# QueensGambit/CrazyAra

Hardware: AMD Instinct MI355X
Metric: nn_evals_per_sec (higher is better)
Workload: dtype f16x3; 1 GPU; crazyhouse RISEv2 19-block (34x8x8 planes -> 5184 policy + value), batch=256, inputs resident in HBM, random-init seeded weights; batch=256, parallelism=replicas x1, precision=float16x3

## Files before the change

crazyara_amd/csrc/nn/kernels.h:

```cpp
#pragma once
#include <hip/hip_runtime.h>
#include <cstdint>

namespace cra {

typedef _Float16 half_t;

constexpr int kSquares = 64;

inline int64_t packed_weight_elems(int cout_pad, int k_total) { return int64_t(cout_pad) * k_total; }

struct ConvArgs {
    const void* x;
    const void* wpk;
    const void* wpk_lo;
    const float* bias;
    const void* resid;
    void* out;
    int batch;
    int cin;
    int cout_pad;
    int cout_real;
    int cout_ld;
    int ks;
    int relu;
    int out_policy_f32;
    int out_flat;
    int flat_pitch;
    int out_rows_f32;
    int rows_valid;
    float* softmax_out;
    const float* planes;
    int planes_c;
    int p8;
    float acc_scale;
    const void *pre_wpk, *pre_wpk_lo;
    const float* pre_bias;
    float pre_acc_scale;
    int dev;
    int few_boards;
    int x_ld;
};

template <typename T> void launch_conv_gemm(const ConvArgs& a, hipStream_t s);

struct BlockArgs {
    const void* x;
    void* y;
    const void* w1pk;
    const float* b1;
    const float* wdw;
    const float* b2;
    const void* w3pk;
    const void* w1pk_lo;
    const void* w3pk_lo;
    const float* b3;
    int batch, C, cop_pad, ks;
    const float* gate;
    float* pool_out;
    const float* dwpk;
};
template <typename T> void launch_block(const BlockArgs& a, hipStream_t s);
void launch_conv_gemm_x3(const ConvArgs& a, hipStream_t s);
void launch_block_x3(const BlockArgs& a, hipStream_t s);
void init_x3_kernel_attributes();
int block_x3_chunk_channels();
struct X3TowerBlock {
    const void *w1pk, *w1pk_lo, *w3pk, *w3pk_lo;
    const float* dwpk;
    const float* b3;
    const float* se_w1t;
    const float* se_w2t;
    const float* se_b;
    int cop_pad;
    int se_kind;
    float w1_inv, w3_scale, w3_inv;
};
struct X3TowerArgs {
    const float* x;
    float* y;
    const X3TowerBlock* blocks;
    int nblocks;
    int batch;
    int p8;
    int ks;
    int symmetric;
};
void launch_tower_x3(const X3TowerArgs& a, hipStream_t s);
struct X3SplitArgs {
    X3TowerBlock blk;
    const float* x_parts;
    float* y_parts;
    int gin;
    int batch, G;
    const float* pool_in;
    float* pool_out;
    int dev;
};
void launch_block_x3_split(const X3SplitArgs& a, hipStream_t s);
void launch_x3_split_finish(const float* parts, int gin, float* y, int batch, hipStream_t s);
template <typename T> void init_block_kernel_attributes();
template <typename T> int block_chunk_channels();

constexpr int kTowerWindow = 16;
struct TowerBlockDesc {
    const float* b3;
    const float* s3;
    const void* se_w1;
    const void* se_w2;
    const float* se_b;
    int cop_pad;
    int ks;
    int se_kind;
    float qx_inv, qt_inv, escale;
};
struct TowerArgs {
    const void* x;
    void* y;
    const TowerBlockDesc* blocks;
    const void* wstream;
    const float* bstream;
    const void* pstream;
    long long wstream_wave_frags, bstream_wave_floats, pstream_wave_bytes;
    int nblocks;
    int batch;
    const float* gate_in;
    float* pool_out;
    unsigned long long* trace;
    int fp8;
    long long wstream_e_frags;
    void* block_dump;
};
void launch_tower(const TowerArgs& a, hipStream_t s);
void init_tower_kernel_attributes();
size_t tower_lds_bytes();
inline int tower_row_of_position(int p) { return (p % 4) + 8 * ((p % 16) / 4) + 4 * (p / 16); }
inline int tower_k_channel(int kpos) {
    const int chunk = kpos / 128, wq = (kpos % 128) / 32, p = kpos % 32;
    return chunk * 128 + wq * 32 + tower_row_of_position(p);
}

struct StemArgs {
    const float* planes;
    void* x;
    const void* stem_w;
    const float* stem_b;
    long long stem_wave_frags;
    int cin, cin_pad;
    int batch;
    const void* descs;
    int layout, n_valid;
};
void launch_stem(const StemArgs& a, hipStream_t s);

struct HeadArgs {
    const void* x;
    float* logits;
    float* probs;
    float* value;
    float* aux;
    const void* s1;
    const float* b1;
    const void* s2;
    long long s1_wave_frags, s2_wave_frags;
    const float* vconv_bias;
    const void* fc1_w;
    const float* fc1_b;
    const float* fc2_w;
    float fc2_b;
    float wdl_b[4];
    int cp;
    int wdlp;
    int batch;
    unsigned long long* trace;
    const uint16_t* g_idx;
    const uint32_t* g_cnt;
    float* g_out;
    int g_stride, g_n_valid;
};
void launch_head(const HeadArgs& a, hipStream_t s);
void init_head_kernel_attributes();
size_t head_lds_bytes();

void launch_forward(const StemArgs& sa, const TowerArgs& ta, const HeadArgs& ha, hipStream_t s);
void init_forward_kernel_attributes();

struct ResTowerArgs {
    const void* x;
    void* y;
    const void* wstream;
    const float* bstream;
    long long wstream_wave_frags;
    long long bstream_wave_floats;
    int nblocks;
    int relu_after_add;
    int batch;
    int boards_per_workgroup;
    int cout_tiles_per_wave;
};
void launch_restower(const ResTowerArgs& a, hipStream_t s);
void init_restower_kernel_attributes();
size_t restower_lds_bytes();

template <typename T> void launch_depthwise(const T* x, T* y, const float* w, const float* bias, int batch, int C, int ks,
                                            hipStream_t s);

template <typename T> void launch_se(T* x, int kind_flags, const float* w1t, const float* w2t, const float* b1, int batch, int C,
                                     hipStream_t s, const T* res = nullptr);

void launch_se_gate(const float* pool, float* gate, int kind, const float* w1t, const float* w2t, const float* b1, int batch, int C,
                    hipStream_t s);

struct ValueHeadArgs {
    const void* x;
    const float* wconv;
    const float* bconv;
    const float* w1t;
    const float* b1;
    const float* w2;
    float b2;
    const float* wwdl;
    const float* bwdl;
    const float* wplys;
    float bplys;
    float* value;
    float* aux;
    int batch, C, cv, fc;
    float* dbg;
    int lds_pad;
    int variant;
};
template <typename T> void prepare_value_head(const ValueHeadArgs& a);
size_t value_head_lds_bytes(const ValueHeadArgs& a);
template <typename T> void launch_value_head(const ValueHeadArgs& a, hipStream_t s);

struct HeadsSmallArgs {
    ConvArgs conv;
    ValueHeadArgs vh;
};
bool heads_small_fits(const ConvArgs& c, const ValueHeadArgs& v);
void launch_heads_small(const HeadsSmallArgs& a, hipStream_t s);
// ... 38 lines not shown
```

crazyara_amd/csrc/nn/precision.cpp:

```cpp
#include <cstdlib>
#include <stdexcept>

#include "rise_net.h"

namespace cra {

namespace {
constexpr bool kX3ValueHeadOneLaunch = true;
}

RiseNet::DevSwitches::DevSwitches() {
    if (const char* e = getenv("CRA_X3_CONV_DEV")) conv_dev = atoi(e);
    device_graph = getenv("CRA_DEVICE_GRAPH") != nullptr;
    lane_graph = getenv("CRA_LANE_GRAPH") != nullptr;
    lane_no_graph = getenv("CRA_LANE_NO_GRAPH") != nullptr;
    predict_copy = getenv("CRA_PREDICT_COPY") != nullptr;
    predict_zero_copy = getenv("CRA_PREDICT_ZERO_COPY") != nullptr;
    if (const char* e = getenv("CRA_LANE_LAUNCHES")) lane_launches = e[0];
    lane_sync = getenv("CRA_LANE_SYNC") != nullptr;
    if (const char* e = getenv("CRA_X3_TOWER")) x3_symmetric = e[0] == 's';
    if (const char* e = getenv("CRA_X3_SPLIT_DEV")) x3_split_dev = atoi(e);
    no_small_path = getenv("CRA_NO_SMALL_PATH") != nullptr;
    if (const char* e = getenv("CRA_SMALL_BATCH_CONV_SPLIT")) small_conv_split = atoi(e);
    tower_trace = getenv("CRA_TOWER_TRACE") != nullptr;
    x3_value_one_launch = kX3ValueHeadOneLaunch;
    if (const char* e = getenv("CRA_X3_VALUE_HEAD")) x3_value_one_launch = e[0] == 'o';
    value_head_debug = getenv("CRA_VALUE_HEAD_DEBUG") != nullptr;
    if (const char* e = getenv("CRA_VALUE_HEAD_LDS_PAD")) value_head_lds_pad = atoi(e);
    if (const char* e = getenv("CRA_VALUE_HEAD_VARIANT")) value_head_variant = atoi(e);
    x3_no_head_chain = getenv("CRA_X3_NO_HEAD_CHAIN") != nullptr;
    small_batch_heads_apart = getenv("CRA_SMALL_BATCH_HEADS_APART") != nullptr;
}

Precision parse_precision(const std::string& precision) {
    Precision v;
    std::string prec = precision;
    auto strip = [&](const std::string& tag) {
        if (prec.size() <= tag.size() || prec.compare(prec.size() - tag.size(), tag.size(), tag) != 0) return false;
        prec.resize(prec.size() - tag.size());
        return true;
    };
    if (strip("-3k")) v.one_launch = false;
    if (strip("-8w")) v.thin_waves = true;
    if (strip("-1wg")) v.board_split = false;
    if (strip("-1b")) v.boards_per_wg = 1;
    else if (strip("-2b")) v.boards_per_wg = 2;
    if (strip("-unfused")) v.fused = v.tower = false;
    else if (strip("-perblock")) v.tower = false;
    using M = Precision::Mode;
    static const std::pair<const char*, M> kModes[] = {
        {"float16", M::Float16},   {"fp16", M::Float16},     {"half", M::Float16},      {"int8", M::Int8},
        {"fp8", M::Fp8},           {"float8", M::Fp8},       {"float32", M::Float32},   {"fp32", M::Float32},
        {"float16x3", M::Float16x3}, {"fp16x3", M::Float16x3}, {"f16x3", M::Float16x3},
        {"float16p8", M::Float16p8}, {"fp16p8", M::Float16p8}, {"f16p8", M::Float16p8}};
    for (const auto& m : kModes)
        if (prec == m.first) {
            v.mode = m.second;
            return v;
        }
    throw std::invalid_argument("unsupported precision '" + precision + "' (float16 | float16x3 | float16p8 | float32 | fp8 | int8)");
}

}
```

crazyara_amd/csrc/nn/rise_net.h:

```cpp
#pragma once
#include <hip/hip_runtime.h>
#include <memory>
#include <string>
#include <utility>
#include <vector>

#include "board_net.h"
#include "netfile.h"

namespace cra {

uint8_t float_to_e4m3(float v);
uint8_t float_to_e5m2(float v);

struct Precision {
    enum class Mode { Float32, Float16, Float16x3, Float16p8, Fp8, Int8 };
    Mode mode = Mode::Float16;
    bool fused = true;
    bool tower = true;
    bool one_launch = true;
    bool thin_waves = false;
    bool board_split = true;
    int boards_per_wg = 0;
    bool fp16() const { return mode == Mode::Float16 || mode == Mode::Fp8 || mode == Mode::Int8; }
    bool x3() const { return mode == Mode::Float16x3 || mode == Mode::Float16p8; }
    bool p8() const { return mode == Mode::Float16p8; }
    bool fp8_tower() const { return mode == Mode::Fp8 || mode == Mode::Int8; }
    bool int8() const { return mode == Mode::Int8; }
};
Precision parse_precision(const std::string& precision);

class RiseNet : public BoardNet {
public:
    RiseNet(const std::string& model_path, int device_id, int batch_size, const std::string& precision) : RiseNet(model_path, device_id, batch_size, precision, nullptr) {}
    ~RiseNet() override;

    const std::string& model_file_path() const { return model_file_path_; }
    bool fp16() const { return prec_.fp16(); }
    int cu_count() const { return cu_count_; }

    void predict(const float* in_planes, float* value, float* probs, float* aux);
    void submit(const float* in_planes, float* value, float* probs, float* aux);
    void wait() override;
    void submit_boards(const void* descs_host, int n_valid, int layout, float* value, float* probs, float* aux, int routing = -1) override;
    void submit_boards_gathered(const void* descs_host, int n_valid, int layout, const uint16_t* idx, const uint32_t* cnt, uint32_t stride,
                                float* value, float* gathered, float* aux, int routing = -1) override;
    struct Group {
        const int* board_of = nullptr;
        int n = 0;
        int layout = 0;
        const void* descs = nullptr;
        const float* planes = nullptr;
        const uint16_t* idx = nullptr;
        const uint32_t* cnt = nullptr;
        uint32_t stride = 0;
        float* gathered = nullptr;
        float* probs = nullptr;
        float* logits = nullptr;
        float* value = nullptr;
        float* aux = nullptr;
    };
    void run_group(const Group& g);

    std::vector<std::pair<float, float>> calibration_maxima(const float* planes_host, int n_boards);

    void keep_logits(bool on) override;
    void* enable_block_dump(int* n_tiles);
    void dev_launch_op(int op, int iters);
    float* value_head_debug() const { return value_head_dbg_; }
    int dev_screen_prepare();
    long dev_screen_run(int op, int launches, long* words);
    std::string dev_screen_info(int op) const;
    void forward_async();

    int launches_per_forward() const { return launches_; }
    const char* op_name(int i) const;
    void time_ops(int iters, float* ms);
    float time_forward(int iters);

    struct IoOverride {
        const float* planes = nullptr;
        float* value = nullptr;
        float* probs = nullptr;
        float* aux = nullptr;
    };
    bool last_submit_was_zero_copy() const { return last_zero_copy_; }

private:
    friend class ExpertSet;
    struct ForwardCall {
        int boards = 0;
        const IoOverride* io = nullptr;
        int prev_g = 1;
    };
    RiseNet(const std::string& model_path, int device_id, int batch_size, const std::string& precision, const RiseNet* parent);
    struct Impl;
    template <typename T> struct Builder;
    template <typename T> void build(const NetFile& nf);
    template <typename T> void enqueue(hipStream_t s, ForwardCall call);
    template <typename T> void launch_op(int i, hipStream_t s, ForwardCall& call);
    void launch_forward_in_stream(ForwardCall call);
    void forward_on(hipStream_t s, ForwardCall call);
    int boards_of_call(int n_valid) const;
    void capture();
    bool buffers_are_pinned(const float* in_planes, float* value, float* probs, float* aux);
    bool last_zero_copy_ = false;
    bool counted_in_flight_ = false;
    int staged_calls_left_ = 0;
    struct DevSwitches {
        int conv_dev = -1;
        bool device_graph = false;
        bool lane_graph = false;
        bool lane_no_graph = false;
        bool predict_copy = false;
        bool predict_zero_copy = false;
        char lane_launches = 0;
        bool lane_sync = false;
        bool x3_symmetric = false;
        int x3_split_dev = 0;
        bool no_small_path = false;
        int small_conv_split = 2;
        bool tower_trace = false;
        bool x3_value_one_launch;
        bool value_head_debug = false;
        int value_head_lds_pad = -1;
        int value_head_variant = 0;
        bool x3_no_head_chain = false;
        bool small_batch_heads_apart = false;
        DevSwitches();
    } dev_;
    float* value_head_dbg_ = nullptr;

    std::string model_file_path_;
    Precision prec_;
    std::vector<std::pair<float, float>> int8_calib_;
    static constexpr int kBoardSplitMaxBatch = 64;
    std::unique_ptr<RiseNet> small_;
    bool owns_stream_ = true;
    int stream_slot_ = -1;
    std::string precision_arg_;
    int cu_count_ = 256;
    int launches_ = 0;
    hipGraph_t graph_ = nullptr;
    hipGraphExec_t graph_exec_ = nullptr;
    void* d_desc_ = nullptr;
    std::unique_ptr<Impl> impl_;
};

std::string int8_calibration_path(const std::string& model_file_path);
std::vector<std::pair<float, float>> read_int8_calibration(const std::string& model_file_path);
std::string calibrate_int8(const std::string& model_path, int device_id, const float* planes_host, int n_boards);
std::vector<float> default_calibration_planes(int channels, int version, int* n_boards);

}
```

crazyara_amd/csrc/nn/rise_net_build.hip:

```cpp
#include <algorithm>
#include <cmath>
#include <cstring>
#include <type_traits>

#include "../chess/planes_host.h"
#include "pack.h"
#include "rise_net_impl.h"

namespace cra {

namespace {
enum class Family {
    Tower,
    X3Tower,
    X3Split,
    Fused,
    Layers,
    Transformer
};
struct BlockPlan {
    Family family;
    bool gate_in_kernel;
};
}
// ... 226 lines not shown
    }
    im.ops.push_back(op);
}

template <typename T> void RiseNet::Builder<T>::stem() {
    const int cin_pad16 = std::max(48, round_up(cin, 16));
    if (prec.tower && prec.fused && kHalf && C == 256 && cin_pad16 <= 96 && !transformers) {
        const StemStreams ss = pack_stem(fold_bn(nf, "body_spatial.0.body.0", "body_spatial.0.body.1"), cin, cin_pad16);
        Op op;
        op.kind = OpKind::Stem;
        op.st.planes = net.d_planes_;
        op.st.x = cur;
        op.st.stem_w = im.upload(ss.w);
        op.st.stem_b = im.upload(ss.b);
        op.st.stem_wave_frags = 9 * (cin_pad16 / 16) + 16;
        op.st.cin = cin;
        op.st.cin_pad = cin_pad16;
        op.st.batch = B;
        im.ops.push_back(op);
        macs += double(kSquares) * cin * C * 9;
        return;
    }
    if (!prec.x3()) {
        Op op;
        op.kind = OpKind::PlanesToAct;
        op.x = net.d_planes_;
        op.y = x0;
        op.C = cin;
        im.ops.push_back(op);
    }
    add_conv("body_spatial.0.body.0", "body_spatial.0.body.1", x0, cur, nullptr, cin, cin_pad, C, 3, true, nullptr);
    if (prec.x3()) {
        im.ops.back().from_planes = true;
        im.ops.back().conv.planes_c = cin;
        if (x3_split) im.ops.back().conv.few_boards = dev.small_conv_split;
    }
}

template <typename T> void RiseNet::Builder<T>::dense_tower() {
    const int NR = prec.thin_waves ? 1 : 2;
    std::vector<Folded> f1s, f2s;
    for (size_t i = 0; i < cops.size(); ++i) {
        const std::string p = "body_spatial." + std::to_string(i + 1);
        f1s.push_back(fold_bn(nf, p + ".body.0", p + ".body.1"));
        f2s.push_back(fold_bn(nf, p + ".body.3", p + ".body.4"));
    }
    const ResTowerStreams rs = pack_restower(f1s, f2s, C, NR);
    Op op;
    op.kind = OpKind::ResTower;
    op.rt.x = cur;
    op.rt.y = nxt;
    op.rt.wstream = im.upload(rs.w);
    op.rt.bstream = im.upload(rs.b);
    op.rt.wstream_wave_frags = (long long)(cops.size() * 2 * 9 * 16 * NR + 16);
    op.rt.bstream_wave_floats = (long long)(cops.size() * 64 * NR);
    op.rt.cout_tiles_per_wave = NR;
    op.rt.nblocks = int(cops.size());
    op.rt.relu_after_add = a0_blocks ? 1 : 0;
    op.rt.batch = B;
    op.rt.boards_per_workgroup = prec.boards_per_wg ? prec.boards_per_wg : (B >= 512 ? 2 : 1);
    im.ops.push_back(op);
    macs += double(cops.size()) * 2.0 * kSquares * C * C * 9;
    std::swap(cur, nxt);
}

template <typename T> void RiseNet::Builder<T>::dense_layer_blocks() {
    auto dense_se_op = [&](const SEWeights& se, T* target, const T* res, bool plain_sigmoid) {
        Op op = se_op(se);
        op.kind = OpKind::SE;
        op.y = target;
        op.x = res;
        macs += se.macs;
        if (plain_sigmoid) op.se_kind |= 16;
        im.ops.push_back(op);
    };
    for (size_t i = 0; i < cops.size(); ++i) {
        const std::string p = "body_spatial." + std::to_string(i + 1);
        const SEWeights se = load_se(nf, p, se_types[i], C);
        if (se.kind && !a0_blocks) dense_se_op(se, cur, nullptr, false);
        add_conv(p + ".body.0", p + ".body.1", cur, nxt, nullptr, C, C, C, 3, 1, nullptr);
        T* out = e;
        if (se.kind && a0_blocks) {
            add_conv(p + ".body.3", p + ".body.4", nxt, out, nullptr, C, C, C, 3, 0, nullptr);
            dense_se_op(se, out, cur, true);
        } else {
            add_conv(p + ".body.3", p + ".body.4", nxt, out, cur, C, C, C, 3, a0_blocks ? 1 : 2, nullptr);
        }
        T* old = cur;
        cur = out;
        e = old;
    }
}

template <typename T> void RiseNet::Builder<T>::bottleneck_blocks() {
    for (size_t i = 0; i < cops.size(); ++i) {
        const std::string p = "body_spatial." + std::to_string(i + 1);
        const int cop = cops[i], k = ks[i];
        const BlockPlan bp = plan(i);
        if (bp.family == Family::Transformer) {
            transformer_block(i);
            continue;
        }
        const bool x3_family = bp.family == Family::X3Tower || bp.family == Family::X3Split;
        if (!x3_blocks.empty() && x3_run_ks != k) flush_x3_run();
        TowerBlockDesc td{};
        X3TowerBlock xb{};
        const SEWeights se = load_se(nf, p, se_types[i], C);
        if (se.kind && bp.gate_in_kernel && bp.family == Family::Tower) {
            const auto pk = pack_se_tower(se);
            td.se_kind = se.kind;
            td.se_w1 = im.upload(pk.first);
            if (se.kind == 1) td.se_w2 = im.upload(pk.second);
            else td.se_b = im.upload(se.b);
        } else if (se.kind && bp.gate_in_kernel) {
            const auto pk = pack_se_x3(se, C);
            xb.se_kind = se.kind;
            xb.se_w1t = im.upload(pk.first);
            if (se.kind == 1) xb.se_w2t = im.upload(pk.second);
            else xb.se_b = im.upload(se.b);
        } else if (se.kind) {
            add_se(se_op(se), bp.family == Family::Fused);
        }
        macs += se.macs;
        if (bp.family == Family::Tower) {
            if (prec.int8() && i >= net.int8_calib_.size()) throw std::runtime_error("INT8 calibration file holds fewer blocks than the model");
            const TowerBlockPack pk = pack_tower_block(fold_block(nf, p), C, cop, k, prec.int8() ? 2 : prec.fp8_tower() ? 1 : 0,
                                                       prec.int8() ? net.int8_calib_[i] : std::pair<float, float>{});
            if (!pk.s3.empty()) td.s3 = im.upload(pk.s3);
            td.b3 = im.upload(pk.b3);
            td.qx_inv = pk.qx_inv;
            td.qt_inv = pk.qt_inv;
            td.escale = pk.escale;
            td.cop_pad = round_up(cop, 128);
            td.ks = k;
            if (tower_blocks.empty()) {
                tower_gate = pending_gate;
                pending_gate = nullptr;
            }
            tower_blocks.push_back(td);
            tower_streams.append(pk.s);
        } else if (x3_family) {
            const int cop_pad = round_up(cop, block_x3_chunk_channels());
            const X3BlockPack pk = pack_x3_block(fold_block(nf, p), C, cop, k, cop_pad, prec.p8() && bp.family != Family::X3Split);
            xb.w1pk = im.upload(pk.w1.hi);
            xb.w1pk_lo = im.upload(pk.w1.lo);
            xb.w3pk = im.upload(pk.w3.hi);
            xb.w3pk_lo = im.upload(pk.w3.lo);
            xb.dwpk = im.upload(pk.dw);
            xb.b3 = im.upload(pk.b3);
            xb.w1_inv = float(pk.w1_inv);
            xb.w3_inv = float(pk.w3_inv);
            xb.w3_scale = float(1.0 / pk.w3_inv);
            xb.cop_pad = cop_pad;
            if (x3_blocks.empty()) x3_run_ks = k;
            x3_blocks.push_back(xb);
        } else if (bp.family == Family::Fused) {
            const int cop_pad = round_up(cop, prec.x3() ? block_x3_chunk_channels() : block_chunk_channels<T>());
            const BlockFold bf = fold_block(nf, p);
            Op op;
            op.kind = OpKind::Block;
            BlockArgs& ba = op.blk;
            ba.x = cur;
            ba.y = nxt;
            upload_dense(ba.w1pk, ba.w1pk_lo, bf.expand, cop, C, 1, cop_pad, C);
            upload_dense(ba.w3pk, ba.w3pk_lo, bf.project, C, cop, 1, C, cop_pad);
            ba.b1 = im.upload_d2f(bf.expand.b, cop_pad);
            ba.wdw = im.upload(pack_depthwise_taps(bf.dw, cop, k, cop_pad));
            ba.b2 = im.upload_d2f(bf.dw.b, cop_pad);
            ba.b3 = im.upload_d2f(bf.project.b, C);
            ba.batch = B;
            ba.C = C;
            ba.cop_pad = cop_pad;
            ba.ks = k;
            if (k == 3)
                ba.dwpk = im.upload(prec.x3() ? pack_x3_depthwise_records(bf.expand, bf.dw, cop, cop_pad, 3)
                                             : pack_depthwise_records12(bf.expand, bf.dw, cop, cop_pad));
            ba.gate = pending_gate;
            pending_gate = nullptr;
            prod_op = int(im.ops.size());
            im.ops.push_back(op);
            std::swap(cur, nxt);
        } else {
            add_conv(p + ".body.0", p + ".body.1", cur, e, nullptr, C, C, cop, 1, true, nullptr);
            {
                Folded fd = fold_bn(nf, p + ".body.3", p + ".body.4");
                Op op;
                op.kind = OpKind::Depthwise;
                op.x = e;
                op.y = f;
                op.w0 = im.upload(pack_depthwise_taps(fd, cop, k, cop));
                op.b0 = im.upload_d2f(fd.b);
                op.C = cop;
                op.ks = k;
                im.ops.push_back(op);
                macs += double(kSquares) * cop * k * k;
            }
            add_conv(p + ".body.6", p + ".body.7", f, nxt, cur, cop, cop, C, 1, false, nullptr);
            std::swap(cur, nxt);
            prod_op = -1;
            continue;
        }
        macs += double(kSquares) * cop * (2.0 * C + k * k);
    }
    flush_tower();
    flush_x3_run();
}

template <typename T> void RiseNet::Builder<T>::transformer_block(size_t i) {
    const NtbFold n = fold_ntb(nf, "body_spatial." + std::to_string(i + 1), C);
    const int D = n.D, M = n.M, H = n.H;
    T* xs = nxt;
    conv_op(n.patch, cur, xs, C, C, D, 1, 0).cout_ld = C;
    conv_op(n.qkv, xs, e, D, D, 3 * D, 1, 0).x_ld = C;
    {
        Op op;
        op.kind = OpKind::Attention;
        op.x = e;
        op.y = f;
        op.C = D;
        im.ops.push_back(op);
    }
    {
        ConvArgs& c = conv_op(n.proj, f, xs, D, D, D, 1, 0);
        c.resid = xs;
        c.cout_ld = C;
    }
    {
        ConvArgs& c = conv_op(n.projection, xs, xs + D, D, D, M, 1, 0);
        c.x_ld = C;
        c.cout_ld = C;
    }
    conv_op(n.mhca, xs + D, f, M, M, M, 3, 1).x_ld = C;
    {
        ConvArgs& c = conv_op(n.mhca_proj, f, xs + D, M, M, M, 1, 0);
        c.resid = xs + D;
        c.cout_ld = C;
    }
    conv_op(n.mlp1, xs, e, C, C, H, 1, 1);
    conv_op(n.mlp2, e, cur, H, H, C, 1, 0).resid = xs;
    macs += n.macs;
    prod_op = -1;
}

template <typename T> void RiseNet::Builder<T>::flush_tower() {
    if (tower_blocks.empty()) return;
    Op op;
    op.kind = OpKind::Tower;
    op.tw.x = cur;
    op.tw.y = nxt;
    op.tw.blocks = im.upload(tower_blocks);
    op.tw.nblocks = int(tower_blocks.size());
    const TowerImage ti = close_tower_streams(std::move(tower_streams), prec.fp8_tower());
    tower_streams = TowerStreams();
    if (prec.fp8_tower()) {
        op.tw.fp8 = prec.int8() ? 2 : 1;
        op.tw.wstream_e_frags = ti.e_frags;
        op.tw.wstream = im.upload(ti.w8);
    } else {
        op.tw.wstream = im.upload(ti.w);
    }
    op.tw.bstream = im.upload(ti.b);
    op.tw.pstream = im.upload(ti.p);
    op.tw.wstream_wave_frags = ti.w_wave_frags;
    op.tw.bstream_wave_floats = ti.b_wave_floats;
    op.tw.pstream_wave_bytes = ti.p_wave_bytes;
    op.tw.batch = B;
    op.tw.gate_in = tower_gate;
    if (dev.tower_trace) op.tw.trace = static_cast<unsigned long long*>(im.dalloc(2 * 256 * sizeof(unsigned long long)));
    prod_op = int(im.ops.size());
    im.ops.push_back(op);
    tower_blocks.clear();
    tower_gate = nullptr;
    std::swap(cur, nxt);
}

template <typename T> void RiseNet::Builder<T>::flush_x3_run() {
    if (x3_blocks.empty()) return;
    if (x3_split && x3_run_ks == 3) {
        if (!split_parts[0])
            for (auto& q : split_parts) q = static_cast<float*>(im.dalloc(size_t(B) * kSplitMaxG * kSquares * C * sizeof(float)));
        const int max_g = std::max(1, std::min(int(kSplitMaxG), net.cu_count_ / B));
        const int nb = int(x3_blocks.size());
        int gin = 1;
        for (int k = 0; k < nb; ++k) {
            Op op;
            op.kind = OpKind::BlockX3Split;
            op.xs.blk = x3_blocks[k];
            op.xs.x_parts = k == 0 ? reinterpret_cast<const float*>(cur) : split_parts[k % 2];
            op.xs.y_parts = split_parts[(k + 1) % 2];
            op.xs.gin = gin;
            op.xs.batch = B;
            op.xs.G = std::min(max_g, x3_blocks[k].cop_pad / block_x3_chunk_channels());
            op.xs.dev = dev.x3_split_dev;
            if (k > 0 && x3_blocks[k].se_kind != 0 && !(dev.x3_split_dev & 8)) {
                float* pools = static_cast<float*>(im.dalloc(size_t(B) * kSplitMaxG * C * sizeof(float)));
                im.ops.back().xs.pool_out = pools;
                op.xs.pool_in = pools;
            }
            gin = op.xs.G;
            im.ops.push_back(op);
        }
        Op fin;
        fin.kind = OpKind::X3SplitFinish;
        fin.xs.x_parts = split_parts[nb % 2];
        fin.xs.gin = gin;
        fin.xs.batch = B;
        fin.xs_y = reinterpret_cast<float*>(nxt);
        im.ops.push_back(fin);
    } else {
        Op op;
        op.kind = OpKind::TowerX3;
        op.tx.x = reinterpret_cast<const float*>(cur);
        op.tx.y = reinterpret_cast<float*>(nxt);
        op.tx.blocks = im.upload(x3_blocks);
        op.tx.nblocks = int(x3_blocks.size());
        op.tx.batch = B;
        op.tx.p8 = prec.p8() ? 1 : 0;
        op.tx.ks = x3_run_ks;
        op.tx.symmetric = dev.x3_symmetric ? 1 : 0;
        im.ops.push_back(op);
    }
    x3_blocks.clear();
    prod_op = -1;
    std::swap(cur, nxt);
}

template <typename T> void RiseNet::Builder<T>::one_launch_head() {
    const Folded fv = fold_bn(nf, "value_head.body.0", "value_head.body.1");
    const HeadStreams hs = pack_head(fold_bn(nf, "policy_head.body.0", "policy_head.body.1"), fold_bn(nf, "policy_head.body.3", ""), fv, C, cv, cp);
    Op op;
    op.kind = OpKind::Head;
    HeadArgs& h = op.hd;
    h.x = cur;
    h.logits = net.d_logits_;
    h.probs = net.d_probs_;
    h.value = net.d_value_;
    h.aux = net.d_aux_;
    h.s1 = im.upload(hs.s1);
    h.b1 = im.upload(hs.b1);
    h.s2 = im.upload(hs.s2);
    h.s1_wave_frags = 9 * 16 + 16 + 16;
    h.s2_wave_frags = 18 * 3 + 9;
    h.vconv_bias = im.upload_d2f(fv.b, 8);
    h.cp = cp;
    h.batch = B;
    if (dev.tower_trace) h.trace = static_cast<unsigned long long*>(im.dalloc(64 * sizeof(unsigned long long)));
    const int nfl = kSquares * cv;
    if (wdl) {
        h.fc1_w = im.upload(pack_value_wdl(nf, nfl, 512));
        const float* bw = nf.get("value_head.body_wdl.0.bias").data;
        h.wdl_b[0] = bw[0]; h.wdl_b[1] = bw[1]; h.wdl_b[2] = bw[2];
        h.wdl_b[3] = nf.get("value_head.body_plys.0.bias").data[0];
        h.wdlp = 1;
        macs += 4.0 * nfl;
    } else {
        const TensorView& w2 = nf.get("value_head.body_final.2.weight");
        const float* bb = nf.get("value_head.body_final.0.bias").data;
        h.fc1_w = im.upload(pack_value_fc1_threads(nf, nfl, fc));
        h.fc1_b = im.upload(std::vector<float>(bb, bb + fc));
        h.fc2_w = im.upload(std::vector<float>(w2.data, w2.data + fc));
        h.fc2_b = nf.get("value_head.body_final.2.bias").data[0];
        macs += double(nfl) * fc + fc;
    }
    macs += double(kSquares) * 9 * (double(C) * C + double(C) * cp) + double(kSquares) * C * cv;
    im.ops.push_back(op);
}

template <typename T> void RiseNet::Builder<T>::policy_head() {
    const bool head_chain = prec.p8() && policy_map && C == 256 && round_up(cp, 16) <= 128 && !x3_split;
    const bool head_chain_x3 = prec.x3() && !prec.p8() && prec.fused && policy_map && C == 256 && round_up(cp, 16) <= 128 && !x3_split &&
                               !dev.x3_no_head_chain;
    if (head_chain || head_chain_x3) {
        Folded f1 = fold_bn(nf, "policy_head.body.0", "policy_head.body.1");
        double inv1 = 1.0;
        SplitPack s1 = head_chain ? pack_dense_p8(f1, C, C, 3, C, C, &inv1) : pack_dense_split(f1, C, C, 3, C, C);
        add_conv("policy_head.body.3", "", cur, nullptr, nullptr, C, C, cp, 3, false, net.d_logits_, head_chain);
        ConvArgs& c = im.ops.back().conv;
        c.pre_wpk = im.upload(s1.hi);
        c.pre_wpk_lo = im.upload(s1.lo);
        c.pre_bias = im.upload_d2f(f1.b, C);
        c.pre_acc_scale = float(inv1);
        macs += double(kSquares) * C * C * 9;
        return;
    }
    add_conv("policy_head.body.0", "policy_head.body.1", cur, nxt, nullptr, C, C, C, 3, true, nullptr, !x3_split);
    im.ops.back().conv.few_boards = x3_split ? dev.small_conv_split : 0;
    if (policy_map) {
        add_conv("policy_head.body.3", "", nxt, nullptr, nullptr, C, C, cp, 3, false, net.d_logits_, !x3_split);
        return;
    }
    const int nfl = cp * kSquares, Bpad = round_up(B, 64);
    T* pflat = static_cast<T*>(im.dalloc(size_t(Bpad) * nfl * sizeof(T)));
    HIP_CHECK(hipMemset(pflat, 0, size_t(Bpad) * nfl * sizeof(T)));
    ConvArgs& c1 = conv_op(fold_bn(nf, "policy_head.body.3", "policy_head.body2.0"), nxt, pflat, C, C, cp, 3, 1);
    c1.out_flat = 1;
    c1.flat_pitch = nfl;
    macs += double(kSquares) * C * cp * 9;
    const TensorView& w = nf.get("policy_head.body3.0.weight");
    const float* bb = nf.get("policy_head.body3.0.bias").data;
    Folded fl;
    fl.w.assign(w.data, w.data + size_t(n_labels) * nfl);
    fl.b.assign(bb, bb + n_labels);
    ConvArgs& c2 = conv_op(fl, pflat, net.d_logits_, nfl, nfl, n_labels, 1, 0);
    c2.batch = Bpad / 64;
    c2.out_rows_f32 = 1;
    c2.rows_valid = B;
    macs += double(nfl) * n_labels;
}

template <typename T> void RiseNet::Builder<T>::softmax() {
    if (prec.x3() && !im.ops.empty() && im.ops.back().kind == OpKind::Conv && im.ops.back().conv.out_policy_f32 &&
        im.ops.back().conv.cout_pad <= 256 && im.ops.back().conv.cout_real * kSquares <= 8192) {
        im.ops.back().fused_softmax = true;
    } else {
        Op op;
        op.kind = OpKind::Softmax;
        im.ops.push_back(op);
    }
}

template <typename T> void RiseNet::Builder<T>::value_head() {
    const bool x3_value_one_launch = prec.x3() && prec.fused && dev.x3_value_one_launch;
    const int nfl = kSquares * cv;
    if (prec.fused && !x3_value_one_launch) {
        const int Bpad = round_up(B, 64);
        T* vflat = static_cast<T*>(im.dalloc(size_t(Bpad) * nfl * sizeof(T)));
        HIP_CHECK(hipMemset(vflat, 0, size_t(Bpad) * nfl * sizeof(T)));
        ConvArgs& c = conv_op(fold_bn(nf, "value_head.body.0", "value_head.body.1"), cur, vflat, C, C, cv, 1, 1);
        c.out_flat = 1;
        c.flat_pitch = nfl;
        macs += double(kSquares) * C * cv;
        Op fin;
        fin.kind = OpKind::ValueFinal;
        ValueFinalArgs& vf = fin.vf;
        vf.value = net.d_value_;
        vf.aux = net.d_aux_;
        vf.batch = B;
        if (wdl) {
            const float* bw = nf.get("value_head.body_wdl.0.bias").data;
            vf.in = vflat;
            vf.n = nfl;
            vf.w = im.upload(pack_value_wdl(nf, nfl, nfl));
            vf.b[0] = bw[0]; vf.b[1] = bw[1]; vf.b[2] = bw[2];
            vf.b[3] = nf.get("value_head.body_plys.0.bias").data[0];
            vf.wdlp = 1;
            macs += 4.0 * nfl;
        } else {
            if (nfl % 32 != 0) throw std::runtime_error("value head flatten size must be a multiple of 32");
            const TensorView &w1 = nf.get("value_head.body_final.0.weight"), &w2 = nf.get("value_head.body_final.2.weight");
            const float* b1 = nf.get("value_head.body_final.0.bias").data;
            Folded f1;
            f1.w.assign(w1.data, w1.data + size_t(fc) * nfl);
            f1.b.assign(b1, b1 + fc);
            const int fc_pad = round_up(fc, 16);
            T* vh = static_cast<T*>(im.dalloc(size_t(Bpad) * fc_pad * sizeof(T)));
            conv_op(f1, vflat, vh, nfl, nfl, fc, 1, 1).batch = Bpad / 64;
            vf.in = vh;
            vf.n = fc_pad;
            std::vector<float> w2p(fc_pad, 0.f);
            std::copy(w2.data, w2.data + fc, w2p.begin());
            vf.w = im.upload(w2p);
            vf.b[0] = nf.get("value_head.body_final.2.bias").data[0];
            vf.wdlp = 0;
            macs += double(nfl) * fc + fc;
        }
        im.ops.push_back(fin);
        return;
    }
    Folded fd = fold_bn(nf, "value_head.body.0", "value_head.body.1");
    Op op;
    op.kind = OpKind::ValueHead;
    ValueHeadArgs& v = op.vh;
// ... 95 lines not shown
```

crazyara_amd/csrc/nn/x3.hip:

```cpp
#include "kernels.h"
#include "device_utils.h"
#include "value_head_body.h"

#include <algorithm>
#include <cstdlib>
#include <stdexcept>
#include <type_traits>

#ifndef CRA_X3_ABL
#define CRA_X3_ABL 0
#endif
#ifndef X3_SGB_VALU
#define X3_SGB_VALU 10
#endif
#if CRA_X3_ABL != 0 && !defined(CRA_DEVELOPMENT)
#error "CRA_X3_ABL is a development switch (wrong results): build with -DCRA_DEVELOPMENT"
#endif
#if defined(CRA_X3_TRACE) && !defined(CRA_DEVELOPMENT)
#error "CRA_X3_TRACE is a development switch: build with -DCRA_DEVELOPMENT"
#endif

namespace cra {

#ifdef CRA_X3_TRACE
__device__ unsigned long long x3_trace[2][8][128][2];
#define X3_STAMP(id)                                                                                    \
    do {                                                                                                \
        if (tracing && trace_n < 128) {                                                                 \
            const unsigned long long t_ = __builtin_readcyclecounter();                                 \
            if (lane == 0) {                                                                            \
                x3_trace[b != 0][wave][trace_n][0] = t_;                                                \
                x3_trace[b != 0][wave][trace_n][1] = (unsigned long long)((kk + 1) * 16 + (id));        \
            }                                                                                           \
            ++trace_n;                                                                                  \
        }                                                                                               \
    } while (0)
#define X3_STAMP_SLAB(i_, sl_) do { const int kk = (i_) - 1; X3_STAMP(6); (void)(sl_); } while (0)
#else
#define X3_STAMP(id) do { } while (0)
#define X3_STAMP_SLAB(i_, sl_) do { } while (0)
#endif

namespace {
constexpr int X3_ABL = CRA_X3_ABL;
__device__ __forceinline__ void x3_mfma(const half8& a, const half8& b, f32x4& c, bool on) {
    if (on) c = __builtin_amdgcn_mfma_f32_16x16x32_f16(a, b, c, 0, 0, 0);
    else asm volatile("" : "+v"(c) : "v"(a), "v"(b));
}

__device__ __forceinline__ void split_pair(float a, float b, uint32_t& hi, uint32_t& lo) {
    float ra, rb;
    asm("v_cvt_pk_f16_f32 %0, %3, %4\n\t"
        "v_fma_mix_f32 %1, %0, -1.0, %3 op_sel_hi:[1,0,0]\n\t"
        "v_fma_mix_f32 %2, %0, -1.0, %4 op_sel:[1,0,0] op_sel_hi:[1,0,0]"
        : "=&v"(hi), "=&v"(ra), "=&v"(rb)
        : "v"(a), "v"(b));
    asm("v_cvt_pk_f16_f32 %0, %1, %2" : "=v"(lo) : "v"(ra), "v"(rb));
}
__device__ __forceinline__ void split8(const float (&v)[8], half8& hi, half8& lo) {
    uint32_t h[4], l[4];
#pragma unroll
    for (int j = 0; j < 4; ++j) split_pair(v[2 * j], v[2 * j + 1], h[j], l[j]);
    typedef uint32_t u32x4 __attribute__((ext_vector_type(4)));
    hi = __builtin_bit_cast(half8, u32x4{h[0], h[1], h[2], h[3]});
    lo = __builtin_bit_cast(half8, u32x4{l[0], l[1], l[2], l[3]});
}
__device__ __forceinline__ void split4(const float (&v)[4], half4& hi, half4& lo) {
    uint32_t h[2], l[2];
#pragma unroll
    for (int j = 0; j < 2; ++j) split_pair(v[2 * j], v[2 * j + 1], h[j], l[j]);
    typedef uint32_t u32x2 __attribute__((ext_vector_type(2)));
    hi = __builtin_bit_cast(half4, u32x2{h[0], h[1]});
    lo = __builtin_bit_cast(half4, u32x2{l[0], l[1]});
}

typedef int i32x4_x3 __attribute__((ext_vector_type(4)));
typedef int i32x8_x3 __attribute__((ext_vector_type(8)));
__device__ __forceinline__ uint32_t x3_high_bytes(uint32_t p01, uint32_t p23) {
    return __builtin_amdgcn_perm(p23, p01, 0x07050301u);
}
__device__ __forceinline__ void split4_b8(const float (&v)[4], half4& hi, uint32_t& h8, uint32_t& l8) {
    uint32_t h[2], l[2];
#pragma unroll
    for (int j = 0; j < 2; ++j) split_pair(v[2 * j], v[2 * j + 1], h[j], l[j]);
    typedef uint32_t u32x2 __attribute__((ext_vector_type(2)));
    hi = __builtin_bit_cast(half4, u32x2{h[0], h[1]});
    h8 = x3_high_bytes(h[0], h[1]);
    l8 = x3_high_bytes(l[0], l[1]);
}
__device__ __forceinline__ void x3_mfma8(const i32x8_x3& a, const i32x8_x3& b, f32x4& c, bool on) {
    if (on) c = __builtin_amdgcn_mfma_scale_f32_16x16x128_f8f6f4(a, b, c, 1, 1, 0, 0, 0, 0);
    else asm volatile("" : "+v"(c) : "v"(a), "v"(b));
}
__device__ __forceinline__ i32x8_x3 x3_cat(const half8& lo16, const half8& hi16) {
    return __builtin_shufflevector(__builtin_bit_cast(i32x4_x3, lo16), __builtin_bit_cast(i32x4_x3, hi16), 0, 1, 2, 3, 4, 5, 6, 7);
}

__device__ __forceinline__ float fmac_shr1(float acc, float x, float w) { return fmaf(w, dpp_mov<DPP_ROW_SHR1>(x), acc); }
__device__ __forceinline__ float fmac_shl1(float acc, float x, float w) { return fmaf(w, dpp_mov<DPP_ROW_SHL1>(x), acc); }

__device__ __forceinline__ void mma_x3(const half8& ah, const half8& al, const half8& bh, const half8& bl, f32x4& c) {
    c = __builtin_amdgcn_mfma_f32_16x16x32_f16(al, bh, c, 0, 0, 0);
    c = __builtin_amdgcn_mfma_f32_16x16x32_f16(ah, bl, c, 0, 0, 0);
    c = __builtin_amdgcn_mfma_f32_16x16x32_f16(ah, bh, c, 0, 0, 0);
}

constexpr int X3_KC = 128;
constexpr int X3_ROWP = X3_KC + 8;

}

template <int MT, int NW>
__device__ __forceinline__ void conv_x3_finish(const ConvArgs& a, f32x4 (&acc)[MT][4], const bool (&active)[MT], char* smem, int b, int co_tile0, float acc_scale) {
    constexpr int NTHR = 64 * NW;
    const int tid = threadIdx.x;
    const int wave = tid >> 6, lane = tid & 63;
    const int l15 = lane & 15, lg = lane >> 4;
    if (a.softmax_out) __syncthreads();
#pragma unroll
    for (int m = 0; m < MT; ++m) {
        if (!active[m]) continue;
        const int co0 = (co_tile0 + m) * 16 + lg * 4;
        float bs[4];
#pragma unroll
        for (int r = 0; r < 4; ++r) bs[r] = a.bias[co0 + r];
#pragma unroll
        for (int t = 0; t < 4; ++t) {
            const int sq = t * 16 + l15;
            float v[4];
#pragma unroll
            for (int r = 0; r < 4; ++r) v[r] = fmaf(acc[m][t][r], acc_scale, bs[r]);
            if (a.relu == 2) {
#pragma unroll
                for (int r = 0; r < 4; ++r) v[r] = fmaxf(v[r], 0.f);
            }
            if (a.resid) {
                float rv[4];
                load4<float>(reinterpret_cast<const float*>(a.resid) + (size_t(b) * kSquares + sq) * a.cout_ld + co0, rv);
#pragma unroll
                for (int r = 0; r < 4; ++r) v[r] += rv[r];
            }
            if (a.relu == 1) {
#pragma unroll
                for (int r = 0; r < 4; ++r) v[r] = fmaxf(v[r], 0.f);
            }
            if (a.out_policy_f32) {
                float* o = reinterpret_cast<float*>(a.out) + size_t(b) * a.cout_real * kSquares;
                float* lds_logits = reinterpret_cast<float*>(smem);
#pragma unroll
                for (int r = 0; r < 4; ++r)
                    if (co0 + r < a.cout_real) {
                        if (a.out) o[(co0 + r) * kSquares + sq] = v[r];
                        if (a.softmax_out) lds_logits[(co0 + r) * kSquares + sq] = v[r];
                    }
            } else if (a.out_rows_f32) {
                const int row = b * kSquares + sq;
                if (row < a.rows_valid) {
                    float* o = reinterpret_cast<float*>(a.out) + size_t(row) * a.cout_real;
#pragma unroll
                    for (int r = 0; r < 4; ++r)
                        if (co0 + r < a.cout_real) o[co0 + r] = v[r];
                }
            } else if (a.out_flat) {
                float* o = reinterpret_cast<float*>(a.out) + size_t(b) * a.flat_pitch;
#pragma unroll
                for (int r = 0; r < 4; ++r)
                    if (co0 + r < a.cout_real) o[(co0 + r) * kSquares + sq] = v[r];
            } else {
                store4<float>(reinterpret_cast<float*>(a.out) + (size_t(b) * kSquares + sq) * a.cout_ld + co0, v);
            }
        }
    }
    if (a.softmax_out) {
        __syncthreads();
        const float* in = reinterpret_cast<const float*>(smem);
        float* red = reinterpret_cast<float*>(smem) + 8192;
        const int n = a.cout_real * kSquares;
        float* out = a.softmax_out + size_t(b) * n;
        float m = -INFINITY;
        for (int i = tid; i < n; i += NTHR) m = fmaxf(m, in[i]);
#pragma unroll
        for (int off = 32; off > 0; off >>= 1) m = fmaxf(m, __shfl_xor(m, off, 64));
        if (lane == 0) red[wave] = m;
        __syncthreads();
        m = red[0];
#pragma unroll
        for (int i = 1; i < NW; ++i) m = fmaxf(m, red[i]);
        float sum = 0.f;
        for (int i = tid; i < n; i += NTHR) sum += expf(in[i] - m);
#pragma unroll
        for (int off = 32; off > 0; off >>= 1) sum += __shfl_xor(sum, off, 64);
        __syncthreads();
        if (lane == 0) red[wave] = sum;
        __syncthreads();
        sum = red[0];
#pragma unroll
        for (int i = 1; i < NW; ++i) sum += red[i];
        const float c = m + logf(sum);
        for (int i = tid; i < n; i += NTHR) out[i] = expf(in[i] - c);
    }
}

template <int KS, int MT, int NW, int NS>
__device__ __forceinline__ void conv_gemm_x3_body(const ConvArgs& a, char* smem, const int bx, const int b) {
    half_t* xh = reinterpret_cast<half_t*>(smem);
    half_t* xl = xh + 65 * X3_ROWP;
    constexpr int ROWP = X3_ROWP, KC = X3_KC, NTHR = 64 * NW;

    const int tid = threadIdx.x;
    const int wave = tid >> 6, lane = tid & 63;
    const int l15 = lane & 15, lg = lane >> 4;
    const int co_tile0 = (bx * NW + wave) * MT;
    bool active[MT];
#pragma unroll
    for (int m = 0; m < MT; ++m) active[m] = (co_tile0 + m) * 16 < a.cout_pad;
    const int x_ld = a.x_ld ? a.x_ld : a.cin;
    const float* xb = reinterpret_cast<const float*>(a.x) + size_t(b) * kSquares * x_ld;
    const int nslab_ci = a.cin >> 5;
    const int nslab = KS * KS * nslab_ci;
    const half8 *wph[MT], *wpl[MT];
#pragma unroll
    for (int m = 0; m < MT; ++m) {
        wph[m] = reinterpret_cast<const half8*>(a.wpk) + size_t(active[m] ? co_tile0 + m : 0) * nslab * 64 + lane;
        wpl[m] = reinterpret_cast<const half8*>(a.wpk_lo) + size_t(active[m] ? co_tile0 + m : 0) * nslab * 64 + lane;
    }

    f32x4 acc[MT][4];
// ... 455 lines not shown
    __device__ __forceinline__ void request(const float* xb, int cin, int kc0, int tid) {
#pragma unroll
        for (int j = 0; j < NV; ++j) {
            const int i = tid + j * 512, r = i / (ConvX3::KC / 8), v = i - r * (ConvX3::KC / 8);
            load8<float>(xb + size_t(r) * cin + kc0 + v * 8, pre[j]);
        }
    }
    __device__ __forceinline__ void split_store(half_t* xh, half_t* xl, int tid) {
#pragma unroll
        for (int j = 0; j < NV; ++j) {
            const int i = tid + j * 512, r = i / (ConvX3::KC / 8), v = i - r * (ConvX3::KC / 8);
            half8 h, l;
            split8(pre[j], h, l);
            *reinterpret_cast<half8*>(xh + r * ConvX3::ROWP + v * 8) = h;
            *reinterpret_cast<half8*>(xl + r * ConvX3::ROWP + v * 8) = l;
        }
    }
};
}

__global__ __launch_bounds__(512) void conv3x3_x3_chain_kernel(const ConvArgs a) {
    extern __shared__ __attribute__((aligned(16))) char smem[];
    constexpr int KC = ConvX3::KC, ROWP = ConvX3::ROWP, NW = 8, C = 256;
    const int b = blockIdx.y;
    const int tid = threadIdx.x;
    const int wave = tid >> 6, lane = tid & 63;
    const int l15 = lane & 15, lg = lane >> 4;
    const float* xb = reinterpret_cast<const float*>(a.x) + size_t(b) * kSquares * C;
    constexpr int nslab_ci = C >> 5, nslab = 9 * nslab_ci;
    {
        const half8 *wph[2], *wpl[2];
#pragma unroll
        for (int m = 0; m < 2; ++m) {
            wph[m] = reinterpret_cast<const half8*>(a.pre_wpk) + size_t(wave * 2 + m) * nslab * 64 + lane;
            wpl[m] = reinterpret_cast<const half8*>(a.pre_wpk_lo) + size_t(wave * 2 + m) * nslab * 64 + lane;
        }
        f32x4 acc[2][4];
#pragma unroll
        for (int m = 0; m < 2; ++m)
#pragma unroll
            for (int t = 0; t < 4; ++t) acc[m][t] = f32x4{0.f, 0.f, 0.f, 0.f};
        for (int i = tid; i < 4 * ROWP; i += 512) {
            const int tile = i / ROWP, c = i - tile * ROWP;
            (tile & 1 ? ConvX3::xl_of(smem, tile >> 1) : ConvX3::xh_of(smem, tile >> 1))[64 * ROWP + c] = half_t(0.f);
        }
        ConvX3Stage stage;
        stage.request(xb, C, 0, tid);
        stage.split_store(ConvX3::xh_of(smem, 0), ConvX3::xl_of(smem, 0), tid);
#pragma unroll 1
        for (int pass = 0; pass < 2; ++pass) {
            const int kc0 = pass * KC;
            ConvX3Window<2> W;
            conv_x3_prime<2>(W, wph, wpl, kc0, nslab_ci);
            __syncthreads();
            if (pass == 0) stage.request(xb, C, KC, tid);
            conv_x3_pass<2>(W, ConvX3::xh_of(smem, pass), ConvX3::xl_of(smem, pass), wph, wpl, kc0, nslab_ci, l15, lg, acc);
            if (pass == 0) stage.split_store(ConvX3::xh_of(smem, 1), ConvX3::xl_of(smem, 1), tid);
        }
        __syncthreads();
#pragma unroll
        for (int m = 0; m < 2; ++m) {
            const int c0 = (wave * 2 + m) * 16 + lg * 4;
            const f32x4 bs = *reinterpret_cast<const f32x4*>(a.pre_bias + c0);
            half_t* xh = ConvX3::xh_of(smem, c0 >> 7);
            half_t* xl = ConvX3::xl_of(smem, c0 >> 7);
#pragma unroll
            for (int t = 0; t < 4; ++t) {
                const int sq = t * 16 + l15;
                float v[4];
#pragma unroll
                for (int r = 0; r < 4; ++r) v[r] = fmaxf(fmaf(acc[m][t][r], 1.f, bs[r]), 0.f);
                half4 h, l;
                split4(v, h, l);
                *reinterpret_cast<half4*>(xh + sq * ROWP + (c0 & 127)) = h;
                *reinterpret_cast<half4*>(xl + sq * ROWP + (c0 & 127)) = l;
            }
        }
    }
    bool active[1] = {wave * 16 < a.cout_pad};
    const half8 *wph[1], *wpl[1];
    wph[0] = reinterpret_cast<const half8*>(a.wpk) + size_t(active[0] ? wave : 0) * nslab * 64 + lane;
    wpl[0] = reinterpret_cast<const half8*>(a.wpk_lo) + size_t(active[0] ? wave : 0) * nslab * 64 + lane;
    f32x4 acc2[1][4];
#pragma unroll
    for (int t = 0; t < 4; ++t) acc2[0][t] = f32x4{0.f, 0.f, 0.f, 0.f};
    ConvX3Window<1> W;
    if (active[0]) conv_x3_prime<1>(W, wph, wpl, 0, nslab_ci);
    __syncthreads();
    if (active[0]) {
#pragma unroll 1
        for (int pass = 0; pass < 2; ++pass) {
            if (pass == 1) conv_x3_prime<1>(W, wph, wpl, KC, nslab_ci);
            conv_x3_pass<1>(W, ConvX3::xh_of(smem, pass), ConvX3::xl_of(smem, pass), wph, wpl, pass * KC, nslab_ci, l15, lg, acc2);
        }
    }
    conv_x3_finish<1, NW>(a, acc2, active, smem, b, wave, 1.f);
}

static void launch_conv3x3_p8(const ConvArgs& a, hipStream_t s) {
    if (a.ks != 3 || a.cin % X3_KC != 0 || a.planes || a.out_rows_f32) throw std::invalid_argument("conv3x3_p8_kernel: a dense 3x3 conv with cin a multiple of 128");
    const size_t shmem = ConvP8::lds_bytes;
    const int tiles = a.cout_pad / 16;
    if (a.pre_wpk) {
        if (a.cin != 256 || tiles > 8 || a.resid) throw std::invalid_argument("conv3x3_p8_chain_kernel: 256 -> 256 -> at most 128 couts, no shortcut");
        hipLaunchKernelGGL(conv3x3_p8_chain_kernel, dim3(1, a.batch), dim3(512), shmem, s, a);
        return;
    }
    if ((tiles >= 12 && !a.few_boards) || (a.softmax_out && tiles > 8)) hipLaunchKernelGGL((conv3x3_p8_kernel<2, 8>), dim3((tiles + 15) / 16, a.batch), dim3(512), shmem, s, a);
    else hipLaunchKernelGGL((conv3x3_p8_kernel<1, 8>), dim3((tiles + 7) / 8, a.batch), dim3(512), shmem, s, a);
}
template <int KS, int NS> static void launch_conv_gemm_x3_ks(const ConvArgs& a, hipStream_t s) {
    const size_t shmem = size_t(2) * 65 * X3_ROWP * sizeof(half_t);
    const int tiles = a.cout_pad / 16;
    if (a.out_rows_f32) {
        hipLaunchKernelGGL((conv_gemm_x3_kernel<KS, 1, 4, NS>), dim3((tiles + 3) / 4, a.batch), dim3(256), shmem, s, a);
    } else if (a.few_boards >= 2 && tiles >= 8 && !a.softmax_out) {
        hipLaunchKernelGGL((conv_gemm_x3_kernel<KS, 1, 4, NS>), dim3((tiles + 3) / 4, a.batch), dim3(256), shmem, s, a);
    } else if ((tiles >= 12 && !a.few_boards) || (a.softmax_out && tiles > 8)) {
        hipLaunchKernelGGL((conv_gemm_x3_kernel<KS, 2, 8, NS>), dim3((tiles + 15) / 16, a.batch), dim3(512), shmem, s, a);
    } else if (tiles >= 5) {
        hipLaunchKernelGGL((conv_gemm_x3_kernel<KS, 1, 8, NS>), dim3((tiles + 7) / 8, a.batch), dim3(512), shmem, s, a);
    } else {
        hipLaunchKernelGGL((conv_gemm_x3_kernel<KS, 1, 4, NS>), dim3((tiles + 3) / 4, a.batch), dim3(256), shmem, s, a);
    }
}
template <int KS> static void launch_conv_gemm_x3_cin(const ConvArgs& a, hipStream_t s) {
    if (a.cin % X3_KC == 0) launch_conv_gemm_x3_ks<KS, X3_KC / 32>(a, s);
    else if (a.cin == 64) launch_conv_gemm_x3_ks<KS, 2>(a, s);
    else launch_conv_gemm_x3_ks<KS, 0>(a, s);
}
void launch_conv_gemm_x3(const ConvArgs& a, hipStream_t s) {
    if (a.pre_wpk && !a.p8) {
        if (a.ks != 3 || a.cin != 256 || a.cout_pad > 128 || a.resid || a.planes || a.out_rows_f32 || !a.out_policy_f32)
            throw std::invalid_argument("conv3x3_x3_chain_kernel: 256 -> 256 -> at most 128 couts of a policy map, no shortcut");
        hipLaunchKernelGGL(conv3x3_x3_chain_kernel, dim3(1, a.batch), dim3(512), ConvX3::lds_bytes, s, a);
        return;
    }
    if (a.p8) launch_conv3x3_p8(a, s);
    else if (a.ks == 1) launch_conv_gemm_x3_cin<1>(a, s);
    else launch_conv_gemm_x3_cin<3>(a, s);
}
bool heads_small_fits(const ConvArgs& c, const ValueHeadArgs& v) {
    return !c.p8 && c.ks == 3 && c.cin % X3_KC == 0 && !c.planes && !c.out_rows_f32 && c.out_policy_f32 && !c.resid && c.cout_pad <= 128 && !v.dbg && v.lds_pad < 0 &&
           v.variant == 0 && value_head_lds_bytes(v) <= 64 * 1024;
}
void launch_heads_small(const HeadsSmallArgs& a, hipStream_t s) {
    if (!heads_small_fits(a.conv, a.vh) || !a.conv.softmax_out || a.conv.batch != a.vh.batch) throw std::invalid_argument("heads_small_kernel: a 3x3 policy conv of at most 128 couts with its softmax, and the one-launch value head");
    const size_t shmem = std::max(size_t(2) * 65 * X3_ROWP * sizeof(half_t), value_head_lds_bytes(a.vh));
    const dim3 grid(16 * ((a.conv.batch + 7) / 8));
    hipLaunchKernelGGL(heads_small_kernel, grid, dim3(512), shmem, s, a);
}

namespace {
struct X3Block {
    static constexpr int C = 256, NW = 8, NE = 1, CK = 16 * NW * NE, NTHR = 64 * NW, NJ = C / 16 / NW;
    static constexpr int XROW = C + 16;
    static constexpr int TROW = CK + 16;
    static constexpr size_t dws_bytes = size_t(NW) * NE * 1024;
    static constexpr int T2BUF = NE == 1 ? 2 : 1;
    static constexpr size_t lds_bytes = (size_t(2) * 64 * XROW + size_t(2) * T2BUF * 64 * TROW) * sizeof(half_t) + dws_bytes;
};
static_assert(X3Block::lds_bytes + 8192 <= 160 * 1024, "LDS budget (tower_p8_kernel<5> takes 8 KiB more for its records)");

struct X3Tiles {
    half_t *xh, *xl;
    half_t *t2h, *t2l;
    float* dws;
};
__device__ __forceinline__ X3Tiles x3_tiles(char* smem) {
    X3Tiles t;
    t.xh = reinterpret_cast<half_t*>(smem);
    t.xl = t.xh + 64 * X3Block::XROW;
    t.t2h = t.xl + 64 * X3Block::XROW;
    t.t2l = t.t2h + X3Block::T2BUF * 64 * X3Block::TROW;
    t.dws = reinterpret_cast<float*>(t.t2l + X3Block::T2BUF * 64 * X3Block::TROW);
    return t;
}

__device__ __forceinline__ int x3_row(int sq) { return ((sq >> 3) & 3) * 16 + (sq >> 5) * 8 + (sq & 7); }
__device__ __forceinline__ int x3_square(int row) { return ((row >> 4) + 4 * ((row >> 3) & 1)) * 8 + (row & 7); }

typedef float f32x2 __attribute__((ext_vector_type(2)));
template <int CTRL> __device__ __forceinline__ f32x2 dpp_mov2(f32x2 v) { return f32x2{dpp_mov<CTRL>(v.x), dpp_mov<CTRL>(v.y)}; }
__device__ __forceinline__ f32x2 pair_of(const f32x4& v, int p) { return p == 0 ? f32x2{v[0], v[1]} : f32x2{v[2], v[3]}; }

struct X3EdgeOffsets { int left, right; };
__device__ __forceinline__ X3EdgeOffsets x3_edge_offsets(int l15) { return X3EdgeOffsets{(l15 & 7) == 0 ? 11 * 16 : 0, (l15 & 7) == 7 ? 5 * 16 : 0}; }
struct X3Depthwise {
    f32x2 w[11];
    f32x2 S[6], L[6], R[6];
    float outv[4][4];

    template <int P> __device__ __forceinline__ void load(const float* rec, int lg, const X3EdgeOffsets& e) {
#pragma unroll
        for (int q = 0; q < 11; ++q) w[q] = *reinterpret_cast<const f32x2*>(rec + (q < 3 ? e.left : q >= 6 && q < 9 ? e.right : 0) + q * 16 + lg * 4 + 2 * P);
    }
    template <int P, bool SCALED = false> __device__ __forceinline__ void gather(const f32x4 (&acc)[4], bool upper, int c0 = 0, int c1 = 2, float acc_scale = 1.f) {
        if constexpr (X3_ABL & 1) {
#pragma unroll
            for (int t = 0; t < 4; ++t) S[1 + t] = pair_of(acc[t], P) + w[0];
            return;
        }
#pragma unroll
        for (int c = 0; c < 2; ++c) {
            if (c < c0 || c >= c1) continue;
#pragma unroll
            for (int t = 0; t < 4; ++t) S[1 + t][c] = SCALED ? fmaxf(fmaf(acc[t][2 * P + c], acc_scale, w[9][c]), 0.f) : fmaxf(acc[t][2 * P + c] + w[9][c], 0.f);
            const float across_up = dpp_mov<DPP_ROW_ROR8>(S[4][c]), across_dn = dpp_mov<DPP_ROW_ROR8>(S[1][c]);
            S[0][c] = upper ? across_up : 0.f;
            S[5][c] = upper ? 0.f : across_dn;
#pragma unroll
            for (int j = 0; j < 6; ++j) {
                L[j][c] = dpp_mov<DPP_ROW_SHR1>(S[j][c]);
                R[j][c] = dpp_mov<DPP_ROW_SHL1>(S[j][c]);
            }
        }
    }
    template <int P> __device__ __forceinline__ void taps(int t0, int t1) {
#pragma unroll
        for (int t = 0; t < 4; ++t) {
            if (t < t0 || t >= t1) continue;
#pragma unroll
            for (int c = 0; c < 2; ++c) {
                if constexpr (X3_ABL & 1) {
                    outv[t][2 * P + c] = S[1 + t][c];
                    continue;
                }
                float a = w[10][c];
#pragma unroll
                for (int dy = 0; dy < 3; ++dy) {
                    a = fmaf(w[dy][c], L[t + dy][c], a);
                    a = fmaf(w[3 + dy][c], S[t + dy][c], a);
                    a = fmaf(w[6 + dy][c], R[t + dy][c], a);
                }
                outv[t][2 * P + c] = fmaxf(a, 0.f);
            }
        }
    }
    __device__ __forceinline__ void pin_taps(int t0, int t1, int P) {
#pragma unroll
        for (int t = 0; t < 4; ++t)
#pragma unroll
            for (int c = 0; c < 2; ++c)
                if (t >= t0 && t < t1) asm volatile("" : "+v"(outv[t][2 * P + c]));
    }
};
__device__ __forceinline__ void x3_depthwise(const f32x4 (&acc)[4], const float* rec, int lg, bool upper, const X3EdgeOffsets& e, float (&outv)[4][4]) {
    X3Depthwise dw;
    dw.template load<0>(rec, lg, e);
    dw.template gather<0>(acc, upper);
    dw.template taps<0>(0, 4);
    dw.template load<1>(rec, lg, e);
    dw.template gather<1>(acc, upper);
    dw.template taps<1>(0, 4);
#pragma unroll
    for (int t = 0; t < 4; ++t)
#pragma unroll
        for (int r = 0; r < 4; ++r) outv[t][r] = dw.outv[t][r];
}
struct X3EdgeOffsets5 { int o[5]; };
__device__ __forceinline__ X3EdgeOffsets5 x3_edge_offsets5(int l15) {
    const int f = l15 & 7;
    X3EdgeOffsets5 e;
    e.o[0] = f < 2 ? 27 * 16 : 0;
    e.o[1] = f < 1 ? 22 * 16 : 0;
    e.o[2] = 0;
    e.o[3] = f > 6 ? 12 * 16 : 0;
    e.o[4] = f > 5 ? 7 * 16 : 0;
    return e;
}
struct X3Depthwise5 {
    float w[27];
    float S[8];
    float outv[4][4];

    template <int CH> __device__ __forceinline__ void load(const float* rec, int lg, const X3EdgeOffsets5& e) {
#pragma unroll
        for (int q = 0; q < 27; ++q) w[q] = rec[(q < 25 ? e.o[q / 5] : 0) + q * 16 + lg * 4 + CH];
    }
    template <int CH> __device__ __forceinline__ void gather(const f32x4 (&acc)[4], bool upper, float acc_scale) {
#pragma unroll
        for (int t = 0; t < 4; ++t) S[2 + t] = fmaxf(fmaf(acc[t][CH], acc_scale, w[25]), 0.f);
        const float u3 = dpp_mov<DPP_ROW_ROR8>(S[5]), u2 = dpp_mov<DPP_ROW_ROR8>(S[4]);
        const float d0 = dpp_mov<DPP_ROW_ROR8>(S[2]), d1 = dpp_mov<DPP_ROW_ROR8>(S[3]);
        S[1] = upper ? u3 : 0.f;
        S[0] = upper ? u2 : 0.f;
        S[6] = upper ? 0.f : d0;
        S[7] = upper ? 0.f : d1;
    }
    template <int CH> __device__ __forceinline__ void taps() {
        float a[4];
#pragma unroll
        for (int t = 0; t < 4; ++t) a[t] = w[26];
#pragma unroll
        for (int j = 0; j < 8; ++j) {
            const float v[5] = {dpp_mov<DPP_ROW_SHR2>(S[j]), dpp_mov<DPP_ROW_SHR1>(S[j]), S[j], dpp_mov<DPP_ROW_SHL1>(S[j]), dpp_mov<DPP_ROW_SHL2>(S[j])};
#pragma unroll
            for (int t = 0; t < 4; ++t) {
                const int dy = j - t;
                if (dy < 0 || dy > 4) continue;
#pragma unroll
                for (int g = 0; g < 5; ++g) a[t] = fmaf(w[g * 5 + dy], v[g], a[t]);
            }
        }
#pragma unroll
        for (int t = 0; t < 4; ++t) outv[t][CH] = fmaxf(a[t], 0.f);
    }
};
__device__ __forceinline__ void x3_stage_tile(const X3Tiles& T, const float* xb, const float* g, int tid) {
    constexpr int C = X3Block::C, XROW = X3Block::XROW;
#pragma unroll 1
    for (int i = tid; i < 64 * (C / 8); i += X3Block::NTHR) {
        const int sq = i / (C / 8), v = i - sq * (C / 8), r = x3_row(sq);
        float f[8];
        load8<float>(xb + size_t(sq) * C + v * 8, f);
        if (g) {
            float gv[8];
            load8<float>(g + v * 8, gv);
#pragma unroll
            for (int j = 0; j < 8; ++j) f[j] *= gv[j];
        }
        half8 h, l;
        split8(f, h, l);
        *reinterpret_cast<half8*>(T.xh + r * XROW + v * 8) = h;
        *reinterpret_cast<half8*>(T.xl + r * XROW + v * 8) = l;
    }
}

struct X3Weights {
    __amdgpu_buffer_rsrc_t w1h, w1l, w3h, w3l;
    __amdgpu_buffer_rsrc_t dw;
    int cop_pad;
};
__device__ __forceinline__ __amdgpu_buffer_rsrc_t x3_rsrc(const void* p) {
    const uint64_t v = reinterpret_cast<uint64_t>(p);
    const uint64_t u = (uint64_t(uint32_t(__builtin_amdgcn_readfirstlane(int(uint32_t(v >> 32))))) << 32) |
                       uint32_t(__builtin_amdgcn_readfirstlane(int(uint32_t(v))));
    return __builtin_amdgcn_make_buffer_rsrc(reinterpret_cast<void*>(u), 0, 0x7fffffff, 0x00020000);
}
__device__ __forceinline__ X3Weights x3_weights(const void* w1h, const void* w1l, const void* w3h, const void* w3l, const float* dwpk, int cop_pad) {
    X3Weights W;
    W.w1h = x3_rsrc(w1h); W.w1l = x3_rsrc(w1l); W.w3h = x3_rsrc(w3h); W.w3l = x3_rsrc(w3l);
    W.dw = x3_rsrc(dwpk);
    W.cop_pad = __builtin_amdgcn_readfirstlane(cop_pad);
    return W;
}
__device__ __forceinline__ half8 x3_frag(__amdgpu_buffer_rsrc_t r, uint32_t lane_off, uint32_t frag) {
    typedef uint32_t u32x4 __attribute__((ext_vector_type(4)));
    return __builtin_bit_cast(half8, __builtin_amdgcn_raw_buffer_load_b128(r, lane_off, frag * 1024u, 0));
}
struct X3ExpandWindow { half8 h[X3Block::NE == 1 ? 4 : 2][X3Block::NE], l[X3Block::NE == 1 ? 4 : 2][X3Block::NE]; };
__device__ __forceinline__ void x3_expand_window_request(X3ExpandWindow& E, const X3Weights& W, int ch) {
    constexpr int EW = X3Block::NE == 1 ? 4 : 2, NE = X3Block::NE;
    const int lane = threadIdx.x & 63, wave = __builtin_amdgcn_readfirstlane(int(threadIdx.x) >> 6);
#pragma unroll
    for (int s = 0; s < EW; ++s)
#pragma unroll
        for (int ne = 0; ne < NE; ++ne) {
            const uint32_t f = uint32_t(ch * (X3Block::CK / 16) + wave * NE + ne) * (X3Block::C / 32) + uint32_t(s);
            E.h[s][ne] = x3_frag(W.w1h, uint32_t(lane) * 16u, f);
            E.l[s][ne] = x3_frag(W.w1l, uint32_t(lane) * 16u, f);
        }
}
template <bool PRE = false>
__device__ __forceinline__ void x3_chunks(const X3Tiles& T, const X3Weights& W, f32x4 (&accP)[X3Block::NJ][4], int ch0 = 0, int ch1 = -1,
                                          const X3ExpandWindow* pre = nullptr) {
    using G = X3Block;
    constexpr int C = G::C, CK = G::CK, XROW = G::XROW, TROW = G::TROW, NJ = G::NJ, NE = G::NE;
    const int tid = threadIdx.x, lane = tid & 63, l15 = lane & 15, lg = lane >> 4;
    const int wave = __builtin_amdgcn_readfirstlane(tid >> 6);
    const uint32_t lane_off = uint32_t(lane) * 16u;
    const int nchunk = ch1 < 0 ? W.cop_pad / CK : ch1;
    const int nslab3 = W.cop_pad >> 5;
    const bool hi = l15 >= 8;
    const X3EdgeOffsets edge = x3_edge_offsets(l15);

    constexpr int EW = NE == 1 ? 4 : 2, PW = 2;
    half8 e_h[EW][NE], e_l[EW][NE];
    if constexpr (X3_ABL & 16) {
#pragma unroll
        for (int s = 0; s < EW; ++s)
#pragma unroll
            for (int ne = 0; ne < NE; ++ne) e_h[s][ne] = e_l[s][ne] = *reinterpret_cast<const half8*>(T.xh + lane * 8);
    }
    auto load_expand = [&](int ch, int s) {
        if constexpr (X3_ABL & 16) return;
#pragma unroll
        for (int ne = 0; ne < NE; ++ne) {
            const uint32_t f = uint32_t(ch * (CK / 16) + wave * NE + ne) * (C / 32) + uint32_t(s);
            e_h[s % EW][ne] = x3_frag(W.w1h, lane_off, f);
            e_l[s % EW][ne] = x3_frag(W.w1l, lane_off, f);
        }
    };
    if constexpr (PRE) {
#pragma unroll
        for (int s = 0; s < EW; ++s)
#pragma unroll
            for (int ne = 0; ne < NE; ++ne) { e_h[s][ne] = pre->h[s][ne]; e_l[s][ne] = pre->l[s][ne]; }
    } else {
#pragma unroll
        for (int s = 0; s < EW; ++s) load_expand(ch0, s);
    }
    for (int ch = ch0; ch < nchunk; ++ch) {
        half_t* const t2h = T.t2h + (G::T2BUF == 2 ? (ch & 1) * 64 * TROW : 0);
        half_t* const t2l = T.t2l + (G::T2BUF == 2 ? (ch & 1) * 64 * TROW : 0);
        f32x4 accE[NE][4];
#pragma unroll
        for (int ne = 0; ne < NE; ++ne)
#pragma unroll
            for (int t = 0; t < 4; ++t) accE[ne][t] = f32x4{0.f, 0.f, 0.f, 0.f};
        f32x4 dw_raw[NE];
#pragma unroll
        for (int ne = 0; ne < NE; ++ne)
            dw_raw[ne] = __builtin_bit_cast(f32x4, __builtin_amdgcn_raw_buffer_load_b128(W.dw, lane_off, uint32_t(ch * CK + (wave * NE + ne) * 16) * 64u, 0));
        float* my_dws = T.dws + (wave * NE) * 256;
        auto park_dw = [&]() {
#pragma unroll
            for (int ne = 0; ne < NE; ++ne) *reinterpret_cast<f32x4*>(my_dws + ne * 256 + lane * 4) = dw_raw[ne];
        };
        half8 bh[2][4], bl[2][4];
        auto read_stream = [&](int s, half8 (&h)[4], half8 (&l)[4]) {
#pragma unroll
            for (int t = 0; t < 4; ++t) {
                if constexpr (X3_ABL & 8) {
                    h[t] = e_h[s % EW][0];
                    l[t] = e_l[s % EW][0];
                } else {
                    h[t] = *reinterpret_cast<const half8*>(T.xh + (t * 16 + l15) * XROW + s * 32 + lg * 8);
                    l[t] = *reinterpret_cast<const half8*>(T.xl + (t * 16 + l15) * XROW + s * 32 + lg * 8);
                }
            }
        };
        read_stream(0, bh[0], bl[0]);
#pragma unroll
        for (int s = 0; s < C / 32; ++s) {
            if (s + 1 < C / 32) read_stream(s + 1, bh[(s + 1) & 1], bl[(s + 1) & 1]);
            __builtin_amdgcn_sched_barrier(0);
#pragma unroll
            for (int ne = 0; ne < NE; ++ne)
#pragma unroll
                for (int t = 0; t < 4; ++t) x3_mfma(e_l[s % EW][ne], bh[s & 1][t], accE[ne][t], !(X3_ABL & 2));
#pragma unroll
            for (int ne = 0; ne < NE; ++ne)
#pragma unroll
                for (int t = 0; t < 4; ++t) x3_mfma(e_h[s % EW][ne], bl[s & 1][t], accE[ne][t], !(X3_ABL & 2));
#pragma unroll
            for (int ne = 0; ne < NE; ++ne)
#pragma unroll
                for (int t = 0; t < 4; ++t) x3_mfma(e_h[s % EW][ne], bh[s & 1][t], accE[ne][t], !(X3_ABL & 2));
            if (s + EW < C / 32) load_expand(ch, s + EW);
            if (s == C / 64) park_dw();
            __builtin_amdgcn_sched_barrier(0);
        }
        half8 p_h[PW][NJ], p_l[PW][NJ];
        if constexpr (X3_ABL & 16) {
#pragma unroll
            for (int s2 = 0; s2 < PW; ++s2)
#pragma unroll
                for (int j = 0; j < NJ; ++j) p_h[s2][j] = p_l[s2][j] = *reinterpret_cast<const half8*>(T.xl + lane * 8);
        }
        auto load_project = [&](int s2) {
            if constexpr (X3_ABL & 16) return;
#pragma unroll
            for (int j = 0; j < NJ; ++j) {
                const uint32_t f = uint32_t(wave * NJ + j) * uint32_t(nslab3) + uint32_t(ch * (CK / 32) + s2);
                p_h[s2 % PW][j] = x3_frag(W.w3h, lane_off, f);
                p_l[s2 % PW][j] = x3_frag(W.w3l, lane_off, f);
            }
        };
#pragma unroll
        for (int s2 = 0; s2 < PW; ++s2) load_project(s2);

#pragma unroll
        for (int ne = 0; ne < NE; ++ne) {
            float outv[4][4];
            x3_depthwise(accE[ne], my_dws + ne * 256, lg, hi, edge, outv);
            const int cl = (wave * NE + ne) * 16 + lg * 4;
#pragma unroll
            for (int t = 0; t < 4; ++t) {
                half4 h, l;
                split4(outv[t], h, l);
                if constexpr (X3_ABL & 64) {
                    asm volatile("" ::"v"(h), "v"(l));
                } else {
                    *reinterpret_cast<half4*>(t2h + (t * 16 + l15) * TROW + cl) = h;
                    *reinterpret_cast<half4*>(t2l + (t * 16 + l15) * TROW + cl) = l;
                }
            }
        }
        if constexpr (!(X3_ABL & 32)) __syncthreads();
        if (ch + 1 < nchunk) {
#pragma unroll
            for (int s = 0; s < EW; ++s) load_expand(ch + 1, s);
        }
        auto read_t2 = [&](int s2, half8 (&h)[4], half8 (&l)[4]) {
#pragma unroll
            for (int t = 0; t < 4; ++t) {
                if constexpr (X3_ABL & 8) {
                    h[t] = p_h[s2 % PW][0];
                    l[t] = p_l[s2 % PW][0];
                } else {
                    h[t] = *reinterpret_cast<const half8*>(t2h + (t * 16 + l15) * TROW + s2 * 32 + lg * 8);
                    l[t] = *reinterpret_cast<const half8*>(t2l + (t * 16 + l15) * TROW + s2 * 32 + lg * 8);
                }
            }
        };
        read_t2(0, bh[0], bl[0]);
#pragma unroll
        for (int s2 = 0; s2 < CK / 32; ++s2) {
            if (s2 + 1 < CK / 32) read_t2(s2 + 1, bh[(s2 + 1) & 1], bl[(s2 + 1) & 1]);
            __builtin_amdgcn_sched_barrier(0);
#pragma unroll
            for (int j = 0; j < NJ; ++j)
#pragma unroll
                for (int t = 0; t < 4; ++t) x3_mfma(p_l[s2 % PW][j], bh[s2 & 1][t], accP[j][t], !(X3_ABL & 4));
#pragma unroll
            for (int j = 0; j < NJ; ++j)
#pragma unroll
                for (int t = 0; t < 4; ++t) x3_mfma(p_h[s2 % PW][j], bl[s2 & 1][t], accP[j][t], !(X3_ABL & 4));
#pragma unroll
            for (int j = 0; j < NJ; ++j)
#pragma unroll
                for (int t = 0; t < 4; ++t) x3_mfma(p_h[s2 % PW][j], bh[s2 & 1][t], accP[j][t], !(X3_ABL & 4));
            if (s2 + PW < CK / 32) load_project(s2 + PW);
            __builtin_amdgcn_sched_barrier(0);
        }
        if constexpr (!(X3_ABL & 32) && G::T2BUF == 1) __syncthreads();
    }
}
}

__global__ __launch_bounds__(512) void block_x3_kernel(const BlockArgs a) {
    using G = X3Block;
    constexpr int C = G::C, XROW = G::XROW, NJ = G::NJ;
    extern __shared__ __attribute__((aligned(16))) char smem[];
    const X3Tiles T = x3_tiles(smem);
    const int b = blockIdx.x;
    const int tid = threadIdx.x, wave = tid >> 6, lane = tid & 63, l15 = lane & 15, lg = lane >> 4;
    const X3Weights W = x3_weights(a.w1pk, a.w1pk_lo, a.w3pk, a.w3pk_lo, a.dwpk, a.cop_pad);
    x3_stage_tile(T, reinterpret_cast<const float*>(a.x) + size_t(b) * 64 * C, a.gate ? a.gate + size_t(b) * C : nullptr, tid);
    __syncthreads();

    f32x4 accP[NJ][4];
#pragma unroll
    for (int j = 0; j < NJ; ++j)
#pragma unroll
        for (int t = 0; t < 4; ++t) accP[j][t] = f32x4{0.f, 0.f, 0.f, 0.f};
    x3_chunks(T, W, accP);

    float* yb = reinterpret_cast<float*>(a.y) + size_t(b) * 64 * C;
#pragma unroll
    for (int j = 0; j < NJ; ++j) {
        const int co0 = (wave * NJ + j) * 16 + lg * 4;
        float bs[4];
        load4<float>(a.b3 + co0, bs);
        float pool[4] = {0.f, 0.f, 0.f, 0.f};
#pragma unroll
        for (int t = 0; t < 4; ++t) {
            const int sq = t * 16 + l15;
            float rh[4], rl[4], v[4];
            load4<half_t>(T.xh + sq * XROW + co0, rh);
            load4<half_t>(T.xl + sq * XROW + co0, rl);
#pragma unroll
            for (int r = 0; r < 4; ++r) {
                v[r] = accP[j][t][r] + bs[r] + (rh[r] + rl[r]);
                pool[r] += v[r];
            }
            store4<float>(yb + size_t(x3_square(sq)) * C + co0, v);
        }
        if (a.pool_out) {
#pragma unroll
            for (int r = 0; r < 4; ++r)
#pragma unroll
                for (int off = 8; off > 0; off >>= 1) pool[r] += __shfl_xor(pool[r], off, 64);
            if (l15 == 0) store4<float>(a.pool_out + size_t(b) * C + co0, pool);
        }
    }
}

namespace {
__device__ __forceinline__ void x3_se_fcs(const X3TowerBlock& d, const float* se_mean, float* se_h, float* se_gate, const f32x4 (&wa)[16], const f32x4 (&wb)[16], int tid) {
    constexpr int GRP = 36;
    auto dot32 = [](const f32x4 (&w)[16], const float* v, float& s0, float& s1) {
#pragma unroll
        for (int k4 = 0; k4 < 8; ++k4) {
            const f32x4 m = *reinterpret_cast<const f32x4*>(v + 4 * k4);
            s0 = fmaf(w[2 * k4][0], m[0], s0); s1 = fmaf(w[2 * k4][1], m[0], s1);
            s0 = fmaf(w[2 * k4][2], m[1], s0); s1 = fmaf(w[2 * k4][3], m[1], s1);
            s0 = fmaf(w[2 * k4 + 1][0], m[2], s0); s1 = fmaf(w[2 * k4 + 1][1], m[2], s1);
            s0 = fmaf(w[2 * k4 + 1][2], m[3], s0); s1 = fmaf(w[2 * k4 + 1][3], m[3], s1);
        }
    };
    if (d.se_kind == 1) {
        {
            const int j2 = tid >> 3, kq = tid & 7;
            float s0 = 0.f, s1 = 0.f;
            dot32(wa, se_mean + kq * GRP, s0, s1);
            s0 += dpp_mov<0x111>(s0); s1 += dpp_mov<0x111>(s1);
            s0 += dpp_mov<0x112>(s0); s1 += dpp_mov<0x112>(s1);
            s0 += dpp_mov<0x114>(s0); s1 += dpp_mov<0x114>(s1);
            if (kq == 7) {
                float* h = se_h + (j2 >> 4) * GRP + 2 * (j2 & 15);
                h[0] = fmaxf(s0, 0.f);
                h[1] = fmaxf(s1, 0.f);
            }
        }
        __syncthreads();
        {
            const int c2 = tid >> 2, kq = tid & 3;
            float s0 = 0.f, s1 = 0.f;
            dot32(wb, se_h + kq * GRP, s0, s1);
            s0 += dpp_mov<0x111>(s0); s1 += dpp_mov<0x111>(s1);
            s0 += dpp_mov<0x112>(s0); s1 += dpp_mov<0x112>(s1);
            if (kq == 3) {
                se_gate[2 * c2] = hard_sigmoid(s0);
                se_gate[2 * c2 + 1] = hard_sigmoid(s1);
            }
        }
    } else {
        const int c2 = tid >> 2, kq = tid & 3;
        float s0 = 0.f, s1 = 0.f;
        dot32(wa, se_mean + (2 * kq) * GRP, s0, s1);
        dot32(wb, se_mean + (2 * kq + 1) * GRP, s0, s1);
        s0 += dpp_mov<0x111>(s0); s1 += dpp_mov<0x111>(s1);
        s0 += dpp_mov<0x112>(s0); s1 += dpp_mov<0x112>(s1);
        if (kq == 3) {
            se_gate[2 * c2] = hard_sigmoid(d.se_b[2 * c2] + s0);
            se_gate[2 * c2 + 1] = hard_sigmoid(d.se_b[2 * c2 + 1] + s1);
        }
    }
    __syncthreads();
}
struct X3SeFirstWeights { f32x4 w[16]; };
__device__ __forceinline__ void x3_se_first_weights_request(X3SeFirstWeights& S, const X3TowerBlock& d, int tid) {
    const f32x4* pk = reinterpret_cast<const f32x4*>(d.se_w1t) + tid;
#pragma unroll
    for (int i = 0; i < 16; ++i) S.w[i] = pk[i * 512];
}
__device__ __forceinline__ void x3_se_phase(const X3Tiles& T, const X3TowerBlock& d, float* scratch, int tid, const X3SeFirstWeights* pre_wa = nullptr) {
    constexpr int C = X3Block::C, XROW = X3Block::XROW, GRP = 36;
    float* se_mean = scratch;
    float* se_h = scratch + 8 * GRP;
    float* se_gate = se_h + 4 * GRP;
    f32x4 wa[16], wb[16];
    auto load_thread_weights = [&](const float* base, f32x4 (&dst)[16]) {
        const f32x4* pk = reinterpret_cast<const f32x4*>(base) + tid;
#pragma unroll
        for (int i = 0; i < 16; ++i) dst[i] = pk[i * 512];
    };
    if (pre_wa) {
#pragma unroll
        for (int i = 0; i < 16; ++i) wa[i] = pre_wa->w[i];
        load_thread_weights(d.se_kind == 1 ? d.se_w2t : d.se_w1t + size_t(16) * 512 * 4, wb);
    } else load_thread_weights(d.se_w1t, wa);
    {
        const int lane = tid & 63, wv = tid >> 6, cg = lane >> 4, sg = lane & 15;
        float sum[8] = {0.f, 0.f, 0.f, 0.f, 0.f, 0.f, 0.f, 0.f};
#pragma unroll
        for (int q = 0; q < 4; ++q) {
            float fh[8], fl[8];
            load8<half_t>(T.xh + x3_row(sg * 4 + q) * XROW + wv * 32 + cg * 8, fh);
            load8<half_t>(T.xl + x3_row(sg * 4 + q) * XROW + wv * 32 + cg * 8, fl);
#pragma unroll
            for (int j = 0; j < 8; ++j) sum[j] += fh[j] + fl[j];
        }
#pragma unroll
        for (int j = 0; j < 8; ++j) {
            sum[j] += dpp_mov<0x111>(sum[j]);
            sum[j] += dpp_mov<0x112>(sum[j]);
            sum[j] += dpp_mov<0x114>(sum[j]);
            sum[j] += dpp_mov<0x118>(sum[j]);
        }
        if (sg == 15) {
#pragma unroll
            for (int j = 0; j < 8; ++j) se_mean[wv * GRP + cg * 8 + j] = sum[j] * (1.f / 64.f);
        }
    }
    if (!pre_wa) load_thread_weights(d.se_kind == 1 ? d.se_w2t : d.se_w1t + size_t(16) * 512 * 4, wb);
    __syncthreads();
    x3_se_fcs(d, se_mean, se_h, se_gate, wa, wb, tid);
#pragma unroll 1
    for (int i = tid; i < 64 * (C / 8); i += X3Block::NTHR) {
        const int r = i / (C / 8), v = i - r * (C / 8);
        float fh[8], fl[8], gv[8];
        load8<half_t>(T.xh + r * XROW + v * 8, fh);
        load8<half_t>(T.xl + r * XROW + v * 8, fl);
        load8<float>(se_gate + v * 8, gv);
#pragma unroll
        for (int j = 0; j < 8; ++j) fh[j] = (fh[j] + fl[j]) * gv[j];
        half8 h, l;
        split8(fh, h, l);
        *reinterpret_cast<half8*>(T.xh + r * XROW + v * 8) = h;
        *reinterpret_cast<half8*>(T.xl + r * XROW + v * 8) = l;
    }
    __syncthreads();
}
__device__ __forceinline__ void x3_se_gate_from_mean(const X3TowerBlock& d, float* scratch, int tid) {
    constexpr int GRP = 36;
    f32x4 wa[16], wb[16];
    auto load_thread_weights = [&](const float* base, f32x4 (&dst)[16]) {
        const f32x4* pk = reinterpret_cast<const f32x4*>(base) + tid;
#pragma unroll
        for (int i = 0; i < 16; ++i) dst[i] = pk[i * 512];
    };
    load_thread_weights(d.se_w1t, wa);
    load_thread_weights(d.se_kind == 1 ? d.se_w2t : d.se_w1t + size_t(16) * 512 * 4, wb);
    __syncthreads();
    x3_se_fcs(d, scratch, scratch + 8 * GRP, scratch + 12 * GRP, wa, wb, tid);
}

template <int NJ>
__device__ __forceinline__ void x3_stream_load(f32x4 (&x)[NJ][4], const float* xb, int tile0, int l15, int lg) {
#pragma unroll
    for (int j = 0; j < NJ; ++j)
#pragma unroll
        for (int t = 0; t < 4; ++t) x[j][t] = *reinterpret_cast<const f32x4*>(xb + size_t(x3_square(t * 16 + l15)) * X3Block::C + (tile0 + j) * 16 + lg * 4);
}
template <int NJ>
__device__ __forceinline__ void x3_stream_store(const f32x4 (&x)[NJ][4], float* yb, int tile0, int l15, int lg) {
#pragma unroll
    for (int j = 0; j < NJ; ++j)
#pragma unroll
        for (int t = 0; t < 4; ++t) *reinterpret_cast<f32x4*>(yb + size_t(x3_square(t * 16 + l15)) * X3Block::C + (tile0 + j) * 16 + lg * 4) = x[j][t];
}
template <int NJ>
__device__ __forceinline__ void x3_stream_add_bias(f32x4 (&x)[NJ][4], const float* b3, int tile0, int lg) {
#pragma unroll
    for (int j = 0; j < NJ; ++j) {
        const f32x4 bs = *reinterpret_cast<const f32x4*>(b3 + (tile0 + j) * 16 + lg * 4);
#pragma unroll
        for (int t = 0; t < 4; ++t) x[j][t] += bs;
    }
}
template <int NJ>
__device__ __forceinline__ void x3_stream_write_tiles(const X3Tiles& T, const f32x4 (&x)[NJ][4], int tile0, int l15, int lg) {
#pragma unroll
    for (int j = 0; j < NJ; ++j) {
        const int co0 = (tile0 + j) * 16 + lg * 4;
#pragma unroll
        for (int t = 0; t < 4; ++t) {
            const int rr = t * 16 + l15;
            const float v[4] = {x[j][t][0], x[j][t][1], x[j][t][2], x[j][t][3]};
            half4 h, l;
            split4(v, h, l);
            *reinterpret_cast<half4*>(T.xh + rr * X3Block::XROW + co0) = h;
            *reinterpret_cast<half4*>(T.xl + rr * X3Block::XROW + co0) = l;
        }
    }
}
template <int NJ>
__device__ __forceinline__ void x3_stream_se(const X3Tiles& T, const X3TowerBlock& d, f32x4 (&x)[NJ][4], float* scratch, int tile0, int tid) {
    constexpr int GRP = 36;
    const int lane = tid & 63, l15 = lane & 15, lg = lane >> 4;
#pragma unroll
    for (int j = 0; j < NJ; ++j) {
        float sum[4];
#pragma unroll
        for (int r = 0; r < 4; ++r) sum[r] = (x[j][0][r] + x[j][1][r]) + (x[j][2][r] + x[j][3][r]);
#pragma unroll
        for (int r = 0; r < 4; ++r) {
            sum[r] += dpp_mov<0x111>(sum[r]);
            sum[r] += dpp_mov<0x112>(sum[r]);
            sum[r] += dpp_mov<0x114>(sum[r]);
            sum[r] += dpp_mov<0x118>(sum[r]);
        }
        if (l15 == 15) {
            const int c = (tile0 + j) * 16 + lg * 4;
#pragma unroll
            for (int r = 0; r < 4; ++r) scratch[((c + r) >> 5) * GRP + ((c + r) & 31)] = sum[r] * (1.f / 64.f);
        }
    }
    x3_se_gate_from_mean(d, scratch, tid);
    const float* se_gate = scratch + 12 * GRP;
#pragma unroll
    for (int j = 0; j < NJ; ++j) {
        const f32x4 g = *reinterpret_cast<const f32x4*>(se_gate + (tile0 + j) * 16 + lg * 4);
#pragma unroll
        for (int t = 0; t < 4; ++t) x[j][t] *= g;
    }
    x3_stream_write_tiles<NJ>(T, x, tile0, l15, lg);
    __syncthreads();
}
}

__global__ __launch_bounds__(512) void tower_x3_kernel(const X3TowerArgs a) {
    using G = X3Block;
    constexpr int C = G::C, NJ = G::NJ;
    extern __shared__ __attribute__((aligned(16))) char smem[];
    const X3Tiles T = x3_tiles(smem);
    const int b = blockIdx.x;
    const int tid = threadIdx.x, wave = tid >> 6, lane = tid & 63, l15 = lane & 15, lg = lane >> 4;
    x3_stage_tile(T, a.x + size_t(b) * 64 * C, nullptr, tid);
    f32x4 accX[NJ][4];
    x3_stream_load<NJ>(accX, a.x + size_t(b) * 64 * C, wave * NJ, l15, lg);
    __syncthreads();
    for (int blk = 0; blk < a.nblocks; ++blk) {
        const X3TowerBlock& d = a.blocks[blk];
        if (blk > 0 && d.se_kind != 0) x3_stream_se<NJ>(T, d, accX, reinterpret_cast<float*>(T.t2h), wave * NJ, tid);
        const X3Weights W = x3_weights(d.w1pk, d.w1pk_lo, d.w3pk, d.w3pk_lo, d.dwpk, d.cop_pad);
        x3_stream_add_bias<NJ>(accX, d.b3, wave * NJ, lg);
        x3_chunks(T, W, accX);
        if (blk + 1 < a.nblocks && a.blocks[blk + 1].se_kind == 0) x3_stream_write_tiles<NJ>(T, accX, wave * NJ, l15, lg);
        __syncthreads();
    }
    x3_stream_store<NJ>(accX, a.y + size_t(b) * 64 * C, wave * NJ, l15, lg);
}

namespace {
template <int GIN>
__device__ __forceinline__ void x3_stage_tile_sum(const X3Tiles& T, const float* parts, int gin, int tid, const float* gate = nullptr) {
    constexpr int C = X3Block::C, XROW = X3Block::XROW, IT = 64 * (C / 8) / X3Block::NTHR;
    constexpr int NG = GIN > 0 ? GIN : 16;
    constexpr int FLY = GIN > 0 && GIN <= 2 ? 4 : GIN > 0 && GIN <= 5 ? 2 : 1;
    static_assert(IT % FLY == 0, "passes");
#pragma unroll
    for (int it0 = 0; it0 < IT; it0 += FLY) {
        f32x4 q[FLY][NG][2];
#pragma unroll
        for (int u = 0; u < FLY; ++u) {
            const int i = tid + (it0 + u) * X3Block::NTHR, sq = i / (C / 8), v = i - sq * (C / 8);
            const float* p0 = parts + size_t(sq) * C + v * 8;
#pragma unroll
            for (int g = 0; g < NG; ++g) {
                if (GIN > 0 || g < gin) {
                    const f32x4* p = reinterpret_cast<const f32x4*>(p0 + size_t(g) * 64 * C);
                    q[u][g][0] = p[0];
                    q[u][g][1] = p[1];
                }
            }
        }
#pragma unroll
        for (int u = 0; u < FLY; ++u) {
            const int i = tid + (it0 + u) * X3Block::NTHR, sq = i / (C / 8), v = i - sq * (C / 8), r = x3_row(sq);
            f32x4 s0 = q[u][0][0], s1 = q[u][0][1];
#pragma unroll
            for (int g = 1; g < NG; ++g) {
                if (GIN > 0 || g < gin) {
                    s0 += q[u][g][0];
                    s1 += q[u][g][1];
                }
            }
            float f[8] = {s0[0], s0[1], s0[2], s0[3], s1[0], s1[1], s1[2], s1[3]};
            if (gate) {
                float gv[8];
                load8<float>(gate + v * 8, gv);
#pragma unroll
                for (int j = 0; j < 8; ++j) f[j] *= gv[j];
            }
            half8 h, l;
            split8(f, h, l);
            *reinterpret_cast<half8*>(T.xh + r * XROW + v * 8) = h;
            *reinterpret_cast<half8*>(T.xl + r * XROW + v * 8) = l;
        }
    }
}
}

__global__ __launch_bounds__(512) void block_x3_split_kernel(const X3SplitArgs a) {
    using G = X3Block;
    constexpr int C = G::C, CK = G::CK, XROW = G::XROW, NJ = G::NJ;
    extern __shared__ __attribute__((aligned(16))) char smem[];
    const X3Tiles T = x3_tiles(smem);
    const int G_ = a.G;
    const int xcd = blockIdx.x & 7, jj = blockIdx.x >> 3;
    const int g = jj % G_, b = xcd + 8 * (jj / G_);
    if (b >= a.batch) return;
    const int tid = threadIdx.x, wave = tid >> 6, lane = tid & 63, l15 = lane & 15, lg = lane >> 4;
    const X3TowerBlock& d = a.blk;
    const X3Weights W = x3_weights(d.w1pk, d.w1pk_lo, d.w3pk, d.w3pk_lo, d.dwpk, d.cop_pad);
    const int n = W.cop_pad / CK;
    const int ch0 = __builtin_amdgcn_readfirstlane(g * n / G_), ch1 = __builtin_amdgcn_readfirstlane((g + 1) * n / G_);
    X3ExpandWindow win;
    x3_expand_window_request(win, W, ch0);
    const bool gate_first = d.se_kind != 0 && a.pool_in != nullptr;
    X3SeFirstWeights se_first;
    if (d.se_kind != 0 && !gate_first) x3_se_first_weights_request(se_first, d, tid);
    const float* gate = nullptr;
    if (gate_first) {
        constexpr int GRP = 36;
        float* scratch = reinterpret_cast<float*>(T.t2h);
        float *se_mean = scratch, *se_h = scratch + 8 * GRP, *se_gate = se_h + 4 * GRP;
        f32x4 wa[16], wb[16];
        {
            const f32x4* pa = reinterpret_cast<const f32x4*>(d.se_w1t) + tid;
            const f32x4* pb = reinterpret_cast<const f32x4*>(d.se_kind == 1 ? d.se_w2t : d.se_w1t + size_t(16) * 512 * 4) + tid;
#pragma unroll
            for (int i = 0; i < 16; ++i) wa[i] = pa[i * 512];
#pragma unroll
            for (int i = 0; i < 16; ++i) wb[i] = pb[i * 512];
        }
        if (tid < C) {
            const float* pin = a.pool_in + size_t(b) * a.gin * C + tid;
            float ps[16];
#pragma unroll
            for (int q = 0; q < 16; ++q) ps[q] = q < a.gin ? pin[q * C] : 0.f;
            float sum = ps[0];
#pragma unroll
            for (int q = 1; q < 16; ++q) sum += ps[q];
            se_mean[(tid >> 5) * GRP + (tid & 31)] = sum * (1.f / 64.f);
        }
        __syncthreads();
        x3_se_fcs(d, se_mean, se_h, se_gate, wa, wb, tid);
        gate = se_gate;
    }
    {
        const float* parts = a.x_parts + size_t(b) * a.gin * 64 * C;
        switch (a.gin) {
            case 1: x3_stage_tile_sum<1>(T, parts, 1, tid, gate); break;
            case 2: x3_stage_tile_sum<2>(T, parts, 2, tid, gate); break;
            case 3: x3_stage_tile_sum<3>(T, parts, 3, tid, gate); break;
            case 4: x3_stage_tile_sum<4>(T, parts, 4, tid, gate); break;
            case 5: x3_stage_tile_sum<5>(T, parts, 5, tid, gate); break;
            case 6: x3_stage_tile_sum<6>(T, parts, 6, tid, gate); break;
            case 7: x3_stage_tile_sum<7>(T, parts, 7, tid, gate); break;
            case 8: x3_stage_tile_sum<8>(T, parts, 8, tid, gate); break;
            case 9: x3_stage_tile_sum<9>(T, parts, 9, tid, gate); break;
            case 10: x3_stage_tile_sum<10>(T, parts, 10, tid, gate); break;
            default: x3_stage_tile_sum<0>(T, parts, a.gin, tid, gate); break;
        }
    }
    __syncthreads();
    if (d.se_kind != 0 && !gate_first) x3_se_phase(T, d, reinterpret_cast<float*>(T.t2h), tid, &se_first);
    f32x4 accP[NJ][4];
#pragma unroll
    for (int j = 0; j < NJ; ++j) {
        const f32x4 bs = g == 0 ? *reinterpret_cast<const f32x4*>(d.b3 + (wave * NJ + j) * 16 + lg * 4) : f32x4{0.f, 0.f, 0.f, 0.f};
#pragma unroll
        for (int t = 0; t < 4; ++t) accP[j][t] = bs;
    }
    if (!(a.dev & 4)) x3_chunks<true>(T, W, accP, ch0, ch1, &win);
    float* yb = a.y_parts + (size_t(b) * G_ + g) * 64 * C;
    f32x4 psum[NJ];
#pragma unroll
// ... 601 lines not shown
        const X3TowerBlock& d = a.blocks[blk];
        if (d.se_kind != 0) {
            constexpr int GRP = 36;
#pragma unroll
            for (int j = 0; j < NJ; ++j) {
                float sum[4];
#pragma unroll
                for (int r = 0; r < 4; ++r) sum[r] = (accX[j][0][r] + accX[j][1][r]) + (accX[j][2][r] + accX[j][3][r]);
#pragma unroll
                for (int r = 0; r < 4; ++r) {
                    sum[r] += dpp_mov<0x111>(sum[r]);
                    sum[r] += dpp_mov<0x112>(sum[r]);
                    sum[r] += dpp_mov<0x114>(sum[r]);
                    sum[r] += dpp_mov<0x118>(sum[r]);
                }
                if (l15 == 15) {
                    const int c = (w * NJ + j) * 16 + lg * 4;
#pragma unroll
                    for (int r = 0; r < 4; ++r) se_scratch[((c + r) >> 5) * GRP + ((c + r) & 31)] = sum[r] * (1.f / 64.f);
                }
            }
            x3_se_gate_from_mean(d, se_scratch, tid);
            const float* se_gate = se_scratch + 12 * GRP;
#pragma unroll
            for (int j = 0; j < NJ; ++j) {
                const f32x4 g = *reinterpret_cast<const f32x4*>(se_gate + (w * NJ + j) * 16 + lg * 4);
#pragma unroll
                for (int t = 0; t < 4; ++t) accX[j][t] *= g;
            }
            write_tiles();
            __syncthreads();
        }
        const X3Weights W = x3_weights(d.w1pk, d.w1pk_lo, d.w3pk, d.w3pk_lo, d.dwpk, d.cop_pad);
        const int n = W.cop_pad / CK;
        const int nslab3 = W.cop_pad >> 5;
#ifdef CRA_X3_TRACE
        const bool tracing = (b == 0 || b == 131) && blk == CRA_X3_TRACE;
        int trace_n = 0;
#endif
        half8 p_h[2][NJ];
        i32x8_x3 p_8[NJ];
        auto load_ph = [&](int k, int s2) {
            if constexpr (X3_ABL & 16) return;
#pragma unroll
            for (int j = 0; j < NJ; ++j) p_h[s2 & 1][j] = x3_frag(W.w3h, lane_off, uint32_t(w * NJ + j) * uint32_t(nslab3) + uint32_t(k * (CK / 32) + s2));
        };
        auto load_p8 = [&](int k, int J) {
#pragma unroll
            for (int j = 0; j < NJ; ++j) {
                const uint32_t f = uint32_t(w * NJ + j) * uint32_t(nslab3) + uint32_t(k * (CK / 32) + 2 * J);
                if constexpr (X3_ABL & (16 | 1024)) continue;
                if constexpr (X3_ABL & 512) {
                    const half8 piece = x3_frag(W.w3l, lane_off, f);
                    p_8[j] = x3_cat(piece, piece);
                    continue;
                }
                p_8[j] = x3_cat(x3_frag(W.w3l, lane_off, f), x3_frag(W.w3l, lane_off, f + 1));
            }
        };
        if constexpr (X3_ABL & (16 | 1024)) {
#pragma unroll
            for (int j = 0; j < NJ; ++j) {
                const half8 any = *reinterpret_cast<const half8*>(T.xh + lane * 8 + j * 512);
                p_8[j] = x3_cat(any, any);
                if constexpr (X3_ABL & 16) p_h[0][j] = p_h[1][j] = any;
            }
        }
        {
            const float ps = d.w3_scale;
#pragma unroll
            for (int j = 0; j < NJ; ++j) {
                const f32x4 bs = *reinterpret_cast<const f32x4*>(d.b3 + (w * NJ + j) * 16 + lg * 4) * ps;
#pragma unroll
                for (int t = 0; t < 4; ++t)
#pragma unroll
                    for (int r = 0; r < 4; ++r) accX[j][t][r] = fmaf(accX[j][t][r], ps, bs[r]);
            }
        }
        load_ph(0, 0);
        load_ph(0, 1);
        load_p8(0, 0);
        __syncthreads();
        __syncthreads();
        for (int kk = 0; kk < n; ++kk) {
            X3_STAMP(8);
            half8 bh[2][4];
            i32x8_x3 b8[4];
            auto read_h = [&](int s2) {
                const half_t* const pe = s2 & 1 ? t2h_odd : t2h_even;
#pragma unroll
                for (int t = 0; t < 4; ++t) bh[s2 & 1][t] = *reinterpret_cast<const half8*>(pe + (kk & 1) * 64 * TROW + t * 16 * TROW + (s2 >> 1) * 64);
            };
            auto read_8 = [&](int J) {
                const char* const pj = J ? t2b_j1 : t2b_j0;
#pragma unroll
                for (int t = 0; t < 4; ++t) {
                    const char* pp = pj + (kk & 1) * 64 * T8ROW + t * 16 * T8ROW;
                    b8[t] = x3_cat(*reinterpret_cast<const half8*>(pp), *reinterpret_cast<const half8*>(pp + 32));
                }
            };
            const int knext = kk + 1 < n ? kk + 1 : kk;
            read_h(0);
            read_8(0);
#pragma unroll
            for (int s2 = 0; s2 < CK / 32; ++s2) {
                if (s2 + 1 < CK / 32) read_h(s2 + 1);
                __builtin_amdgcn_sched_barrier(0);
#pragma unroll
                for (int j = 0; j < NJ; ++j)
#pragma unroll
                    for (int t = 0; t < 4; ++t) x3_mfma(p_h[s2 & 1][j], bh[s2 & 1][t], accX[j][t], !(X3_ABL & 4));
                if (s2 & 1) {
#pragma unroll
                    for (int j = 0; j < NJ; ++j)
#pragma unroll
                        for (int t = 0; t < 4; ++t) x3_mfma8(p_8[j], b8[t], accX[j][t], !(X3_ABL & 4));
                    __builtin_amdgcn_sched_barrier(0);
                    if (s2 == 1) { read_8(1); load_p8(kk, 1); } else load_p8(knext, 0);
                }
                if (s2 + 2 < CK / 32) load_ph(kk, s2 + 2); else load_ph(knext, s2 + 2 - CK / 32);
                __builtin_amdgcn_sched_barrier(0);
            }
            X3_STAMP(10);
            if (kk + 1 < n) __syncthreads();
            X3_STAMP(11);
        }
        {
            const float pi = d.w3_inv;
#pragma unroll
            for (int j = 0; j < NJ; ++j)
#pragma unroll
                for (int t = 0; t < 4; ++t) accX[j][t] *= pi;
        }
        const bool next_gated = blk + 1 < a.nblocks && a.blocks[blk + 1].se_kind != 0;
        if (!next_gated) write_tiles();
        { const int kk = n; X3_STAMP(12); }
        __syncthreads();
        { const int kk = n; X3_STAMP(13); }
    }
    float* yb = a.y + size_t(b) * 64 * C;
#pragma unroll
    for (int j = 0; j < NJ; ++j)
#pragma unroll
        for (int t = 0; t < 4; ++t)
            *reinterpret_cast<f32x4*>(yb + size_t(x3_square(t * 16 + l15)) * C + (w * NJ + j) * 16 + lg * 4) = accX[j][t];
}

void init_x3_kernel_attributes() {
    (void)hipFuncSetAttribute(reinterpret_cast<const void*>(&block_x3_kernel), hipFuncAttributeMaxDynamicSharedMemorySize, int(X3Block::lds_bytes));
    (void)hipFuncSetAttribute(reinterpret_cast<const void*>(&tower_x3_kernel), hipFuncAttributeMaxDynamicSharedMemorySize, int(X3Block::lds_bytes));
    (void)hipFuncSetAttribute(reinterpret_cast<const void*>(&block_x3_split_kernel), hipFuncAttributeMaxDynamicSharedMemorySize, int(X3Block::lds_bytes));
    (void)hipFuncSetAttribute(reinterpret_cast<const void*>(&tower_x3_roles_kernel<3>), hipFuncAttributeMaxDynamicSharedMemorySize, int(X3Block::lds_bytes));
    (void)hipFuncSetAttribute(reinterpret_cast<const void*>(&tower_x3_roles_kernel<5>), hipFuncAttributeMaxDynamicSharedMemorySize, int(X3Block::lds_bytes + 8192));
    (void)hipFuncSetAttribute(reinterpret_cast<const void*>(&tower_p8_kernel<3>), hipFuncAttributeMaxDynamicSharedMemorySize, int(X3Block::lds_bytes));
    (void)hipFuncSetAttribute(reinterpret_cast<const void*>(&tower_p8_kernel<5>), hipFuncAttributeMaxDynamicSharedMemorySize, int(X3Block::lds_bytes + 8192));
    (void)hipFuncSetAttribute(reinterpret_cast<const void*>(&conv3x3_x3_chain_kernel), hipFuncAttributeMaxDynamicSharedMemorySize, int(ConvX3::lds_bytes));
    const int conv_p8_lds = int(ConvP8::lds_bytes);
    (void)hipFuncSetAttribute(reinterpret_cast<const void*>(&conv3x3_p8_chain_kernel), hipFuncAttributeMaxDynamicSharedMemorySize, conv_p8_lds);
    (void)hipFuncSetAttribute(reinterpret_cast<const void*>(&conv3x3_p8_kernel<2, 8>), hipFuncAttributeMaxDynamicSharedMemorySize, conv_p8_lds);
    (void)hipFuncSetAttribute(reinterpret_cast<const void*>(&conv3x3_p8_kernel<1, 8>), hipFuncAttributeMaxDynamicSharedMemorySize, conv_p8_lds);
}
int block_x3_chunk_channels() { return X3Block::CK; }

void launch_block_x3(const BlockArgs& a, hipStream_t s) {
    hipLaunchKernelGGL(block_x3_kernel, dim3(a.batch), dim3(X3Block::NTHR), X3Block::lds_bytes, s, a);
}
void launch_block_x3_split(const X3SplitArgs& a, hipStream_t s) {
    const int n = a.blk.cop_pad / X3Block::CK;
    if (a.G < 1 || a.G > n || a.G > 16 || a.gin < 1 || a.gin > 16) throw std::invalid_argument("block_x3_split: 1 <= G <= min(chunks, 16), 1 <= gin <= 16");
    hipLaunchKernelGGL(block_x3_split_kernel, dim3(8 * a.G * ((a.batch + 7) / 8)), dim3(X3Block::NTHR), X3Block::lds_bytes, s, a);
}
void launch_x3_split_finish(const float* parts, int gin, float* y, int batch, hipStream_t s) {
    const int n4 = batch * 64 * X3Block::C / 4;
    hipLaunchKernelGGL(x3_split_finish_kernel, dim3(std::min(1024, (n4 + 255) / 256)), dim3(256), 0, s, parts, gin, y, batch);
}
void launch_tower_x3(const X3TowerArgs& a, hipStream_t s) {
    const bool symmetric = a.symmetric != 0;
    if (a.p8) {
        if (symmetric) throw std::invalid_argument("Precision float16p8 runs the two-role tower only");
        if (a.ks == 5) hipLaunchKernelGGL(tower_p8_kernel<5>, dim3(a.batch), dim3(X3Block::NTHR), X3Block::lds_bytes + 8192, s, a);
        else hipLaunchKernelGGL(tower_p8_kernel<3>, dim3(a.batch), dim3(X3Block::NTHR), X3Block::lds_bytes, s, a);
    } else if (a.ks == 5) {
        hipLaunchKernelGGL(tower_x3_roles_kernel<5>, dim3(a.batch), dim3(X3Block::NTHR), X3Block::lds_bytes + 8192, s, a);
    } else if (symmetric) hipLaunchKernelGGL(tower_x3_kernel, dim3(a.batch), dim3(X3Block::NTHR), X3Block::lds_bytes, s, a);
    else hipLaunchKernelGGL(tower_x3_roles_kernel<3>, dim3(a.batch), dim3(X3Block::NTHR), X3Block::lds_bytes, s, a);
}

}
```

Before: 341,400 evals/s.

## Add half-chunk tail path to x3 tower to skip padded expansion channels

Adds a per-block tail flag set when the padded expansion width exceeds the real width by at least 64 channels. A new tower kernel variant then processes the last chunk at half width, using single-wave expand and depthwise steps and half the projection slabs, so it avoids MFMA work on padding. Shared device helpers move into a separate header, and an environment switch can turn the path off. The cost is more template variants and a more complex schedule, with a risk of register pressure or of the tail chunk being imbalanced across waves.

```diff
diff --git a/crazyara_amd/csrc/nn/kernels.h b/crazyara_amd/csrc/nn/kernels.h
--- a/crazyara_amd/csrc/nn/kernels.h
+++ b/crazyara_amd/csrc/nn/kernels.h
@@ -75,7 +75,9 @@
     int cop_pad;
     int se_kind;
     float w1_inv, w3_scale, w3_inv;
-};
+    int tail;
+};
+static_assert(sizeof(X3TowerBlock) == 96, "the tower kernels index a device array of these");
 struct X3TowerArgs {
     const float* x;
     float* y;
@@ -85,8 +87,11 @@
     int p8;
     int ks;
     int symmetric;
+    int no_tail;
 };
 void launch_tower_x3(const X3TowerArgs& a, hipStream_t s);
+void launch_tower_x3_tail(const X3TowerArgs& a, hipStream_t s);
+void init_x3_tail_kernel_attributes();
 struct X3SplitArgs {
     X3TowerBlock blk;
     const float* x_parts;
diff --git a/crazyara_amd/csrc/nn/precision.cpp b/crazyara_amd/csrc/nn/precision.cpp
--- a/crazyara_amd/csrc/nn/precision.cpp
+++ b/crazyara_amd/csrc/nn/precision.cpp
@@ -29,6 +29,7 @@
     if (const char* e = getenv("CRA_VALUE_HEAD_LDS_PAD")) value_head_lds_pad = atoi(e);
     if (const char* e = getenv("CRA_VALUE_HEAD_VARIANT")) value_head_variant = atoi(e);
     x3_no_head_chain = getenv("CRA_X3_NO_HEAD_CHAIN") != nullptr;
+    x3_no_tail = getenv("CRA_X3_NO_TAIL") != nullptr;
     small_batch_heads_apart = getenv("CRA_SMALL_BATCH_HEADS_APART") != nullptr;
 }
 
diff --git a/crazyara_amd/csrc/nn/rise_net.h b/crazyara_amd/csrc/nn/rise_net.h
--- a/crazyara_amd/csrc/nn/rise_net.h
+++ b/crazyara_amd/csrc/nn/rise_net.h
@@ -126,6 +126,7 @@
         int value_head_lds_pad = -1;
         int value_head_variant = 0;
         bool x3_no_head_chain = false;
+        bool x3_no_tail = false;
         bool small_batch_heads_apart = false;
         DevSwitches();
     } dev_;
diff --git a/crazyara_amd/csrc/nn/rise_net_build.hip b/crazyara_amd/csrc/nn/rise_net_build.hip
--- a/crazyara_amd/csrc/nn/rise_net_build.hip
+++ b/crazyara_amd/csrc/nn/rise_net_build.hip
@@ -402,6 +402,7 @@
             xb.w3_inv = float(pk.w3_inv);
             xb.w3_scale = float(1.0 / pk.w3_inv);
             xb.cop_pad = cop_pad;
+            xb.tail = cop_pad - cop >= 64 ? 1 : 0;
             if (x3_blocks.empty()) x3_run_ks = k;
             x3_blocks.push_back(xb);
         } else if (bp.family == Family::Fused) {
@@ -568,6 +569,7 @@
         op.tx.p8 = prec.p8() ? 1 : 0;
         op.tx.ks = x3_run_ks;
         op.tx.symmetric = dev.x3_symmetric ? 1 : 0;
+        op.tx.no_tail = dev.x3_no_tail ? 1 : 0;
         im.ops.push_back(op);
     }
     x3_blocks.clear();
diff --git a/crazyara_amd/csrc/nn/x3.hip b/crazyara_amd/csrc/nn/x3.hip
--- a/crazyara_amd/csrc/nn/x3.hip
+++ b/crazyara_amd/csrc/nn/x3.hip
@@ -1,78 +1,20 @@
 #include "kernels.h"
 #include "device_utils.h"
 #include "value_head_body.h"
+#include "x3_device.h"
 
 #include <algorithm>
 #include <cstdlib>
 #include <stdexcept>
 #include <type_traits>
 
-#ifndef CRA_X3_ABL
-#define CRA_X3_ABL 0
-#endif
 #ifndef X3_SGB_VALU
 #define X3_SGB_VALU 10
 #endif
-#if CRA_X3_ABL != 0 && !defined(CRA_DEVELOPMENT)
-#error "CRA_X3_ABL is a development switch (wrong results): build with -DCRA_DEVELOPMENT"
-#endif
-#if defined(CRA_X3_TRACE) && !defined(CRA_DEVELOPMENT)
-#error "CRA_X3_TRACE is a development switch: build with -DCRA_DEVELOPMENT"
-#endif
 
 namespace cra {
 
-#ifdef CRA_X3_TRACE
-__device__ unsigned long long x3_trace[2][8][128][2];
-#define X3_STAMP(id)                                                                                    \
-    do {                                                                                                \
-        if (tracing && trace_n < 128) {                                                                 \
-            const unsigned long long t_ = __builtin_readcyclecounter();                                 \
-            if (lane == 0) {                                                                            \
-                x3_trace[b != 0][wave][trace_n][0] = t_;                                                \
-                x3_trace[b != 0][wave][trace_n][1] = (unsigned long long)((kk + 1) * 16 + (id));        \
-            }                                                                                           \
-            ++trace_n;                                                                                  \
-        }                                                                                               \
-    } while (0)
-#define X3_STAMP_SLAB(i_, sl_) do { const int kk = (i_) - 1; X3_STAMP(6); (void)(sl_); } while (0)
-#else
-#define X3_STAMP(id) do { } while (0)
-#define X3_STAMP_SLAB(i_, sl_) do { } while (0)
-#endif
-
 namespace {
-constexpr int X3_ABL = CRA_X3_ABL;
-__device__ __forceinline__ void x3_mfma(const half8& a, const half8& b, f32x4& c, bool on) {
-    if (on) c = __builtin_amdgcn_mfma_f32_16x16x32_f16(a, b, c, 0, 0, 0);
-    else asm volatile("" : "+v"(c) : "v"(a), "v"(b));
-}
-
-__device__ __forceinline__ void split_pair(float a, float b, uint32_t& hi, uint32_t& lo) {
-    float ra, rb;
-    asm("v_cvt_pk_f16_f32 %0, %3, %4\n\t"
-        "v_fma_mix_f32 %1, %0, -1.0, %3 op_sel_hi:[1,0,0]\n\t"
-        "v_fma_mix_f32 %2, %0, -1.0, %4 op_sel:[1,0,0] op_sel_hi:[1,0,0]"
-        : "=&v"(hi), "=&v"(ra), "=&v"(rb)
-        : "v"(a), "v"(b));
-    asm("v_cvt_pk_f16_f32 %0, %1, %2" : "=v"(lo) : "v"(ra), "v"(rb));
-}
-__device__ __forceinline__ void split8(const float (&v)[8], half8& hi, half8& lo) {
-    uint32_t h[4], l[4];
-#pragma unroll
-    for (int j = 0; j < 4; ++j) split_pair(v[2 * j], v[2 * j + 1], h[j], l[j]);
-    typedef uint32_t u32x4 __attribute__((ext_vector_type(4)));
-    hi = __builtin_bit_cast(half8, u32x4{h[0], h[1], h[2], h[3]});
-    lo = __builtin_bit_cast(half8, u32x4{l[0], l[1], l[2], l[3]});
-}
-__device__ __forceinline__ void split4(const float (&v)[4], half4& hi, half4& lo) {
-    uint32_t h[2], l[2];
-#pragma unroll
-    for (int j = 0; j < 2; ++j) split_pair(v[2 * j], v[2 * j + 1], h[j], l[j]);
-    typedef uint32_t u32x2 __attribute__((ext_vector_type(2)));
-    hi = __builtin_bit_cast(half4, u32x2{h[0], h[1]});
-    lo = __builtin_bit_cast(half4, u32x2{l[0], l[1]});
-}
 
 typedef int i32x4_x3 __attribute__((ext_vector_type(4)));
 typedef int i32x8_x3 __attribute__((ext_vector_type(8)));
@@ -834,203 +776,6 @@
 }
 
 namespace {
-struct X3Block {
-    static constexpr int C = 256, NW = 8, NE = 1, CK = 16 * NW * NE, NTHR = 64 * NW, NJ = C / 16 / NW;
-    static constexpr int XROW = C + 16;
-    static constexpr int TROW = CK + 16;
-    static constexpr size_t dws_bytes = size_t(NW) * NE * 1024;
-    static constexpr int T2BUF = NE == 1 ? 2 : 1;
-    static constexpr size_t lds_bytes = (size_t(2) * 64 * XROW + size_t(2) * T2BUF * 64 * TROW) * sizeof(half_t) + dws_bytes;
-};
-static_assert(X3Block::lds_bytes + 8192 <= 160 * 1024, "LDS budget (tower_p8_kernel<5> takes 8 KiB more for its records)");
-
-struct X3Tiles {
-    half_t *xh, *xl;
-    half_t *t2h, *t2l;
-    float* dws;
-};
-__device__ __forceinline__ X3Tiles x3_tiles(char* smem) {
-    X3Tiles t;
-    t.xh = reinterpret_cast<half_t*>(smem);
-    t.xl = t.xh + 64 * X3Block::XROW;
-    t.t2h = t.xl + 64 * X3Block::XROW;
-    t.t2l = t.t2h + X3Block::T2BUF * 64 * X3Block::TROW;
-    t.dws = reinterpret_cast<float*>(t.t2l + X3Block::T2BUF * 64 * X3Block::TROW);
-    return t;
-}
-
-__device__ __forceinline__ int x3_row(int sq) { return ((sq >> 3) & 3) * 16 + (sq >> 5) * 8 + (sq & 7); }
-__device__ __forceinline__ int x3_square(int row) { return ((row >> 4) + 4 * ((row >> 3) & 1)) * 8 + (row & 7); }
-
-typedef float f32x2 __attribute__((ext_vector_type(2)));
-template <int CTRL> __device__ __forceinline__ f32x2 dpp_mov2(f32x2 v) { return f32x2{dpp_mov<CTRL>(v.x), dpp_mov<CTRL>(v.y)}; }
-__device__ __forceinline__ f32x2 pair_of(const f32x4& v, int p) { return p == 0 ? f32x2{v[0], v[1]} : f32x2{v[2], v[3]}; }
-
-struct X3EdgeOffsets { int left, right; };
-__device__ __forceinline__ X3EdgeOffsets x3_edge_offsets(int l15) { return X3EdgeOffsets{(l15 & 7) == 0 ? 11 * 16 : 0, (l15 & 7) == 7 ? 5 * 16 : 0}; }
-struct X3Depthwise {
-    f32x2 w[11];
-    f32x2 S[6], L[6], R[6];
-    float outv[4][4];
-
-    template <int P> __device__ __forceinline__ void load(const float* rec, int lg, const X3EdgeOffsets& e) {
-#pragma unroll
-        for (int q = 0; q < 11; ++q) w[q] = *reinterpret_cast<const f32x2*>(rec + (q < 3 ? e.left : q >= 6 && q < 9 ? e.right : 0) + q * 16 + lg * 4 + 2 * P);
-    }
-    template <int P, bool SCALED = false> __device__ __forceinline__ void gather(const f32x4 (&acc)[4], bool upper, int c0 = 0, int c1 = 2, float acc_scale = 1.f) {
-        if constexpr (X3_ABL & 1) {
-#pragma unroll
-            for (int t = 0; t < 4; ++t) S[1 + t] = pair_of(acc[t], P) + w[0];
-            return;
-        }
-#pragma unroll
-        for (int c = 0; c < 2; ++c) {
-            if (c < c0 || c >= c1) continue;
-#pragma unroll
-            for (int t = 0; t < 4; ++t) S[1 + t][c] = SCALED ? fmaxf(fmaf(acc[t][2 * P + c], acc_scale, w[9][c]), 0.f) : fmaxf(acc[t][2 * P + c] + w[9][c], 0.f);
-            const float across_up = dpp_mov<DPP_ROW_ROR8>(S[4][c]), across_dn = dpp_mov<DPP_ROW_ROR8>(S[1][c]);
-            S[0][c] = upper ? across_up : 0.f;
-            S[5][c] = upper ? 0.f : across_dn;
-#pragma unroll
-            for (int j = 0; j < 6; ++j) {
-                L[j][c] = dpp_mov<DPP_ROW_SHR1>(S[j][c]);
-                R[j][c] = dpp_mov<DPP_ROW_SHL1>(S[j][c]);
-            }
-        }
-    }
-    template <int P> __device__ __forceinline__ void taps(int t0, int t1) {
-#pragma unroll
-        for (int t = 0; t < 4; ++t) {
-            if (t < t0 || t >= t1) continue;
-#pragma unroll
-            for (int c = 0; c < 2; ++c) {
-                if constexpr (X3_ABL & 1) {
-                    outv[t][2 * P + c] = S[1 + t][c];
-                    continue;
-                }
-                float a = w[10][c];
-#pragma unroll
-                for (int dy = 0; dy < 3; ++dy) {
-                    a = fmaf(w[dy][c], L[t + dy][c], a);
-                    a = fmaf(w[3 + dy][c], S[t + dy][c], a);
-                    a = fmaf(w[6 + dy][c], R[t + dy][c], a);
-                }
-                outv[t][2 * P + c] = fmaxf(a, 0.f);
-            }
-        }
-    }
-    __device__ __forceinline__ void pin_taps(int t0, int t1, int P) {
-#pragma unroll
-        for (int t = 0; t < 4; ++t)
-#pragma unroll
-            for (int c = 0; c < 2; ++c)
-                if (t >= t0 && t < t1) asm volatile("" : "+v"(outv[t][2 * P + c]));
-    }
-};
-__device__ __forceinline__ void x3_depthwise(const f32x4 (&acc)[4], const float* rec, int lg, bool upper, const X3EdgeOffsets& e, float (&outv)[4][4]) {
-    X3Depthwise dw;
-    dw.template load<0>(rec, lg, e);
-    dw.template gather<0>(acc, upper);
-    dw.template taps<0>(0, 4);
-    dw.template load<1>(rec, lg, e);
-    dw.template gather<1>(acc, upper);
-    dw.template taps<1>(0, 4);
-#pragma unroll
-    for (int t = 0; t < 4; ++t)
-#pragma unroll
-        for (int r = 0; r < 4; ++r) outv[t][r] = dw.outv[t][r];
-}
-struct X3EdgeOffsets5 { int o[5]; };
-__device__ __forceinline__ X3EdgeOffsets5 x3_edge_offsets5(int l15) {
-    const int f = l15 & 7;
-    X3EdgeOffsets5 e;
-    e.o[0] = f < 2 ? 27 * 16 : 0;
-    e.o[1] = f < 1 ? 22 * 16 : 0;
-    e.o[2] = 0;
-    e.o[3] = f > 6 ? 12 * 16 : 0;
-    e.o[4] = f > 5 ? 7 * 16 : 0;
-    return e;
-}
-struct X3Depthwise5 {
-    float w[27];
-    float S[8];
-    float outv[4][4];
-
-    template <int CH> __device__ __forceinline__ void load(const float* rec, int lg, const X3EdgeOffsets5& e) {
-#pragma unroll
-        for (int q = 0; q < 27; ++q) w[q] = rec[(q < 25 ? e.o[q / 5] : 0) + q * 16 + lg * 4 + CH];
-    }
-    template <int CH> __device__ __forceinline__ void gather(const f32x4 (&acc)[4], bool upper, float acc_scale) {
-#pragma unroll
-        for (int t = 0; t < 4; ++t) S[2 + t] = fmaxf(fmaf(acc[t][CH], acc_scale, w[25]), 0.f);
-        const float u3 = dpp_mov<DPP_ROW_ROR8>(S[5]), u2 = dpp_mov<DPP_ROW_ROR8>(S[4]);
-        const float d0 = dpp_mov<DPP_ROW_ROR8>(S[2]), d1 = dpp_mov<DPP_ROW_ROR8>(S[3]);
-        S[1] = upper ? u3 : 0.f;
-        S[0] = upper ? u2 : 0.f;
-        S[6] = upper ? 0.f : d0;
-        S[7] = upper ? 0.f : d1;
-    }
-    template <int CH> __device__ __forceinline__ void taps() {
-        float a[4];
-#pragma unroll
-        for (int t = 0; t < 4; ++t) a[t] = w[26];
-#pragma unroll
-        for (int j = 0; j < 8; ++j) {
-            const float v[5] = {dpp_mov<DPP_ROW_SHR2>(S[j]), dpp_mov<DPP_ROW_SHR1>(S[j]), S[j], dpp_mov<DPP_ROW_SHL1>(S[j]), dpp_mov<DPP_ROW_SHL2>(S[j])};
-#pragma unroll
-            for (int t = 0; t < 4; ++t) {
-                const int dy = j - t;
-                if (dy < 0 || dy > 4) continue;
-#pragma unroll
-                for (int g = 0; g < 5; ++g) a[t] = fmaf(w[g * 5 + dy], v[g], a[t]);
-            }
-        }
-#pragma unroll
-        for (int t = 0; t < 4; ++t) outv[t][CH] = fmaxf(a[t], 0.f);
-    }
-};
-__device__ __forceinline__ void x3_stage_tile(const X3Tiles& T, const float* xb, const float* g, int tid) {
-    constexpr int C = X3Block::C, XROW = X3Block::XROW;
-#pragma unroll 1
-    for (int i = tid; i < 64 * (C / 8); i += X3Block::NTHR) {
-        const int sq = i / (C / 8), v = i - sq * (C / 8), r = x3_row(sq);
-        float f[8];
-        load8<float>(xb + size_t(sq) * C + v * 8, f);
-        if (g) {
-            float gv[8];
-            load8<float>(g + v * 8, gv);
-#pragma unroll
-            for (int j = 0; j < 8; ++j) f[j] *= gv[j];
-        }
-        half8 h, l;
-        split8(f, h, l);
-        *reinterpret_cast<half8*>(T.xh + r * XROW + v * 8) = h;
-        *reinterpret_cast<half8*>(T.xl + r * XROW + v * 8) = l;
-    }
-}
-
-struct X3Weights {
-    __amdgpu_buffer_rsrc_t w1h, w1l, w3h, w3l;
-    __amdgpu_buffer_rsrc_t dw;
-    int cop_pad;
-};
-__device__ __forceinline__ __amdgpu_buffer_rsrc_t x3_rsrc(const void* p) {
-    const uint64_t v = reinterpret_cast<uint64_t>(p);
-    const uint64_t u = (uint64_t(uint32_t(__builtin_amdgcn_readfirstlane(int(uint32_t(v >> 32))))) << 32) |
-                       uint32_t(__builtin_amdgcn_readfirstlane(int(uint32_t(v))));
-    return __builtin_amdgcn_make_buffer_rsrc(reinterpret_cast<void*>(u), 0, 0x7fffffff, 0x00020000);
-}
-__device__ __forceinline__ X3Weights x3_weights(const void* w1h, const void* w1l, const void* w3h, const void* w3l, const float* dwpk, int cop_pad) {
-    X3Weights W;
-    W.w1h = x3_rsrc(w1h); W.w1l = x3_rsrc(w1l); W.w3h = x3_rsrc(w3h); W.w3l = x3_rsrc(w3l);
-    W.dw = x3_rsrc(dwpk);
-    W.cop_pad = __builtin_amdgcn_readfirstlane(cop_pad);
-    return W;
-}
-__device__ __forceinline__ half8 x3_frag(__amdgpu_buffer_rsrc_t r, uint32_t lane_off, uint32_t frag) {
-    typedef uint32_t u32x4 __attribute__((ext_vector_type(4)));
-    return __builtin_bit_cast(half8, __builtin_amdgcn_raw_buffer_load_b128(r, lane_off, frag * 1024u, 0));
-}
 struct X3ExpandWindow { half8 h[X3Block::NE == 1 ? 4 : 2][X3Block::NE], l[X3Block::NE == 1 ? 4 : 2][X3Block::NE]; };
 __device__ __forceinline__ void x3_expand_window_request(X3ExpandWindow& E, const X3Weights& W, int ch) {
     constexpr int EW = X3Block::NE == 1 ? 4 : 2, NE = X3Block::NE;
@@ -1261,58 +1006,6 @@
 }
 
 namespace {
-__device__ __forceinline__ void x3_se_fcs(const X3TowerBlock& d, const float* se_mean, float* se_h, float* se_gate, const f32x4 (&wa)[16], const f32x4 (&wb)[16], int tid) {
-    constexpr int GRP = 36;
-    auto dot32 = [](const f32x4 (&w)[16], const float* v, float& s0, float& s1) {
-#pragma unroll
-        for (int k4 = 0; k4 < 8; ++k4) {
-            const f32x4 m = *reinterpret_cast<const f32x4*>(v + 4 * k4);
-            s0 = fmaf(w[2 * k4][0], m[0], s0); s1 = fmaf(w[2 * k4][1], m[0], s1);
-            s0 = fmaf(w[2 * k4][2], m[1], s0); s1 = fmaf(w[2 * k4][3], m[1], s1);
-            s0 = fmaf(w[2 * k4 + 1][0], m[2], s0); s1 = fmaf(w[2 * k4 + 1][1], m[2], s1);
-            s0 = fmaf(w[2 * k4 + 1][2], m[3], s0); s1 = fmaf(w[2 * k4 + 1][3], m[3], s1);
-        }
-    };
-    if (d.se_kind == 1) {
-        {
-            const int j2 = tid >> 3, kq = tid & 7;
-            float s0 = 0.f, s1 = 0.f;
-            dot32(wa, se_mean + kq * GRP, s0, s1);
-            s0 += dpp_mov<0x111>(s0); s1 += dpp_mov<0x111>(s1);
-            s0 += dpp_mov<0x112>(s0); s1 += dpp_mov<0x112>(s1);
-            s0 += dpp_mov<0x114>(s0); s1 += dpp_mov<0x114>(s1);
-            if (kq == 7) {
-                float* h = se_h + (j2 >> 4) * GRP + 2 * (j2 & 15);
-                h[0] = fmaxf(s0, 0.f);
-                h[1] = fmaxf(s1, 0.f);
-            }
-        }
-        __syncthreads();
-        {
-            const int c2 = tid >> 2, kq = tid & 3;
-            float s0 = 0.f, s1 = 0.f;
-            dot32(wb, se_h + kq * GRP, s0, s1);
-            s0 += dpp_mov<0x111>(s0); s1 += dpp_mov<0x111>(s1);
-            s0 += dpp_mov<0x112>(s0); s1 += dpp_mov<0x112>(s1);
-            if (kq == 3) {
-                se_gate[2 * c2] = hard_sigmoid(s0);
-                se_gate[2 * c2 + 1] = hard_sigmoid(s1);
-            }
-        }
-    } else {
-        const int c2 = tid >> 2, kq = tid & 3;
-        float s0 = 0.f, s1 = 0.f;
-        dot32(wa, se_mean + (2 * kq) * GRP, s0, s1);
-        dot32(wb, se_mean + (2 * kq + 1) * GRP, s0, s1);
-        s0 += dpp_mov<0x111>(s0); s1 += dpp_mov<0x111>(s1);
-        s0 += dpp_mov<0x112>(s0); s1 += dpp_mov<0x112>(s1);
-        if (kq == 3) {
-            se_gate[2 * c2] = hard_sigmoid(d.se_b[2 * c2] + s0);
-            se_gate[2 * c2 + 1] = hard_sigmoid(d.se_b[2 * c2 + 1] + s1);
-        }
-    }
-    __syncthreads();
-}
 struct X3SeFirstWeights { f32x4 w[16]; };
 __device__ __forceinline__ void x3_se_first_weights_request(X3SeFirstWeights& S, const X3TowerBlock& d, int tid) {
     const f32x4* pk = reinterpret_cast<const f32x4*>(d.se_w1t) + tid;
@@ -1375,92 +1068,6 @@
         *reinterpret_cast<half8*>(T.xh + r * XROW + v * 8) = h;
         *reinterpret_cast<half8*>(T.xl + r * XROW + v * 8) = l;
     }
-    __syncthreads();
-}
-__device__ __forceinline__ void x3_se_gate_from_mean(const X3TowerBlock& d, float* scratch, int tid) {
-    constexpr int GRP = 36;
-    f32x4 wa[16], wb[16];
-    auto load_thread_weights = [&](const float* base, f32x4 (&dst)[16]) {
-        const f32x4* pk = reinterpret_cast<const f32x4*>(base) + tid;
-#pragma unroll
-        for (int i = 0; i < 16; ++i) dst[i] = pk[i * 512];
-    };
-    load_thread_weights(d.se_w1t, wa);
-    load_thread_weights(d.se_kind == 1 ? d.se_w2t : d.se_w1t + size_t(16) * 512 * 4, wb);
-    __syncthreads();
-    x3_se_fcs(d, scratch, scratch + 8 * GRP, scratch + 12 * GRP, wa, wb, tid);
-}
-
-template <int NJ>
-__device__ __forceinline__ void x3_stream_load(f32x4 (&x)[NJ][4], const float* xb, int tile0, int l15, int lg) {
-#pragma unroll
-    for (int j = 0; j < NJ; ++j)
-#pragma unroll
-        for (int t = 0; t < 4; ++t) x[j][t] = *reinterpret_cast<const f32x4*>(xb + size_t(x3_square(t * 16 + l15)) * X3Block::C + (tile0 + j) * 16 + lg * 4);
-}
-template <int NJ>
-__device__ __forceinline__ void x3_stream_store(const f32x4 (&x)[NJ][4], float* yb, int tile0, int l15, int lg) {
-#pragma unroll
-    for (int j = 0; j < NJ; ++j)
-#pragma unroll
-        for (int t = 0; t < 4; ++t) *reinterpret_cast<f32x4*>(yb + size_t(x3_square(t * 16 + l15)) * X3Block::C + (tile0 + j) * 16 + lg * 4) = x[j][t];
-}
-template <int NJ>
-__device__ __forceinline__ void x3_stream_add_bias(f32x4 (&x)[NJ][4], const float* b3, int tile0, int lg) {
-#pragma unroll
-    for (int j = 0; j < NJ; ++j) {
-        const f32x4 bs = *reinterpret_cast<const f32x4*>(b3 + (tile0 + j) * 16 + lg * 4);
-#pragma unroll
-        for (int t = 0; t < 4; ++t) x[j][t] += bs;
-    }
-}
-template <int NJ>
-__device__ __forceinline__ void x3_stream_write_tiles(const X3Tiles& T, const f32x4 (&x)[NJ][4], int tile0, int l15, int lg) {
-#pragma unroll
-    for (int j = 0; j < NJ; ++j) {
-        const int co0 = (tile0 + j) * 16 + lg * 4;
-#pragma unroll
-        for (int t = 0; t < 4; ++t) {
-            const int rr = t * 16 + l15;
-            const float v[4] = {x[j][t][0], x[j][t][1], x[j][t][2], x[j][t][3]};
-            half4 h, l;
-            split4(v, h, l);
-            *reinterpret_cast<half4*>(T.xh + rr * X3Block::XROW + co0) = h;
-            *reinterpret_cast<half4*>(T.xl + rr * X3Block::XROW + co0) = l;
-        }
-    }
-}
-template <int NJ>
-__device__ __forceinline__ void x3_stream_se(const X3Tiles& T, const X3TowerBlock& d, f32x4 (&x)[NJ][4], float* scratch, int tile0, int tid) {
-    constexpr int GRP = 36;
-    const int lane = tid & 63, l15 = lane & 15, lg = lane >> 4;
-#pragma unroll
-    for (int j = 0; j < NJ; ++j) {
-        float sum[4];
-#pragma unroll
-        for (int r = 0; r < 4; ++r) sum[r] = (x[j][0][r] + x[j][1][r]) + (x[j][2][r] + x[j][3][r]);
-#pragma unroll
-        for (int r = 0; r < 4; ++r) {
-            sum[r] += dpp_mov<0x111>(sum[r]);
-            sum[r] += dpp_mov<0x112>(sum[r]);
-            sum[r] += dpp_mov<0x114>(sum[r]);
-            sum[r] += dpp_mov<0x118>(sum[r]);
-        }
-        if (l15 == 15) {
-            const int c = (tile0 + j) * 16 + lg * 4;
-#pragma unroll
-            for (int r = 0; r < 4; ++r) scratch[((c + r) >> 5) * GRP + ((c + r) & 31)] = sum[r] * (1.f / 64.f);
-        }
-    }
-    x3_se_gate_from_mean(d, scratch, tid);
-    const float* se_gate = scratch + 12 * GRP;
-#pragma unroll
-    for (int j = 0; j < NJ; ++j) {
-        const f32x4 g = *reinterpret_cast<const f32x4*>(se_gate + (tile0 + j) * 16 + lg * 4);
-#pragma unroll
-        for (int t = 0; t < 4; ++t) x[j][t] *= g;
-    }
-    x3_stream_write_tiles<NJ>(T, x, tile0, l15, lg);
     __syncthreads();
 }
 }
@@ -2368,6 +1975,7 @@
     (void)hipFuncSetAttribute(reinterpret_cast<const void*>(&block_x3_split_kernel), hipFuncAttributeMaxDynamicSharedMemorySize, int(X3Block::lds_bytes));
     (void)hipFuncSetAttribute(reinterpret_cast<const void*>(&tower_x3_roles_kernel<3>), hipFuncAttributeMaxDynamicSharedMemorySize, int(X3Block::lds_bytes));
     (void)hipFuncSetAttribute(reinterpret_cast<const void*>(&tower_x3_roles_kernel<5>), hipFuncAttributeMaxDynamicSharedMemorySize, int(X3Block::lds_bytes + 8192));
+    init_x3_tail_kernel_attributes();
     (void)hipFuncSetAttribute(reinterpret_cast<const void*>(&tower_p8_kernel<3>), hipFuncAttributeMaxDynamicSharedMemorySize, int(X3Block::lds_bytes));
     (void)hipFuncSetAttribute(reinterpret_cast<const void*>(&tower_p8_kernel<5>), hipFuncAttributeMaxDynamicSharedMemorySize, int(X3Block::lds_bytes + 8192));
     (void)hipFuncSetAttribute(reinterpret_cast<const void*>(&conv3x3_x3_chain_kernel), hipFuncAttributeMaxDynamicSharedMemorySize, int(ConvX3::lds_bytes));
@@ -2396,6 +2004,8 @@
         if (symmetric) throw std::invalid_argument("Precision float16p8 runs the two-role tower only");
         if (a.ks == 5) hipLaunchKernelGGL(tower_p8_kernel<5>, dim3(a.batch), dim3(X3Block::NTHR), X3Block::lds_bytes + 8192, s, a);
         else hipLaunchKernelGGL(tower_p8_kernel<3>, dim3(a.batch), dim3(X3Block::NTHR), X3Block::lds_bytes, s, a);
+    } else if (!symmetric && !a.no_tail) {
+        launch_tower_x3_tail(a, s);
     } else if (a.ks == 5) {
         hipLaunchKernelGGL(tower_x3_roles_kernel<5>, dim3(a.batch), dim3(X3Block::NTHR), X3Block::lds_bytes + 8192, s, a);
     } else if (symmetric) hipLaunchKernelGGL(tower_x3_kernel, dim3(a.batch), dim3(X3Block::NTHR), X3Block::lds_bytes, s, a);
diff --git a/crazyara_amd/csrc/nn/x3_device.h b/crazyara_amd/csrc/nn/x3_device.h
--- /dev/null
+++ b/crazyara_amd/csrc/nn/x3_device.h
@@ -0,0 +1,415 @@
+#pragma once
+#include "kernels.h"
+#include "device_utils.h"
+
+#include <type_traits>
+
+#ifndef CRA_X3_ABL
+#define CRA_X3_ABL 0
+#endif
+#if CRA_X3_ABL != 0 && !defined(CRA_DEVELOPMENT)
+#error "CRA_X3_ABL is a development switch (wrong results): build with -DCRA_DEVELOPMENT"
+#endif
+#if defined(CRA_X3_TRACE) && !defined(CRA_DEVELOPMENT)
+#error "CRA_X3_TRACE is a development switch: build with -DCRA_DEVELOPMENT"
+#endif
+
+namespace cra {
+
+#ifdef CRA_X3_TRACE
+namespace {
+__device__ unsigned long long x3_trace[2][8][128][2];
+}
+#define X3_STAMP(id)                                                                                    \
+    do {                                                                                                \
+        if (tracing && trace_n < 128) {                                                                 \
+            const unsigned long long t_ = __builtin_readcyclecounter();                                 \
+            if (lane == 0) {                                                                            \
+                x3_trace[b != 0][wave][trace_n][0] = t_;                                                \
+                x3_trace[b != 0][wave][trace_n][1] = (unsigned long long)((kk + 1) * 16 + (id));        \
+            }                                                                                           \
+            ++trace_n;                                                                                  \
+        }                                                                                               \
+    } while (0)
+#define X3_STAMP_SLAB(i_, sl_) do { const int kk = (i_) - 1; X3_STAMP(6); (void)(sl_); } while (0)
+#else
+#define X3_STAMP(id) do { } while (0)
+#define X3_STAMP_SLAB(i_, sl_) do { } while (0)
+#endif
+
+namespace {
+constexpr int X3_ABL = CRA_X3_ABL;
+__device__ __forceinline__ void x3_mfma(const half8& a, const half8& b, f32x4& c, bool on) {
+    if (on) c = __builtin_amdgcn_mfma_f32_16x16x32_f16(a, b, c, 0, 0, 0);
+    else asm volatile("" : "+v"(c) : "v"(a), "v"(b));
+}
+
+__device__ __forceinline__ void split_pair(float a, float b, uint32_t& hi, uint32_t& lo) {
+    float ra, rb;
+    asm("v_cvt_pk_f16_f32 %0, %3, %4\n\t"
+        "v_fma_mix_f32 %1, %0, -1.0, %3 op_sel_hi:[1,0,0]\n\t"
+        "v_fma_mix_f32 %2, %0, -1.0, %4 op_sel:[1,0,0] op_sel_hi:[1,0,0]"
+        : "=&v"(hi), "=&v"(ra), "=&v"(rb)
+        : "v"(a), "v"(b));
+    asm("v_cvt_pk_f16_f32 %0, %1, %2" : "=v"(lo) : "v"(ra), "v"(rb));
+}
+__device__ __forceinline__ void split8(const float (&v)[8], half8& hi, half8& lo) {
+    uint32_t h[4], l[4];
+#pragma unroll
+    for (int j = 0; j < 4; ++j) split_pair(v[2 * j], v[2 * j + 1], h[j], l[j]);
+    typedef uint32_t u32x4 __attribute__((ext_vector_type(4)));
+    hi = __builtin_bit_cast(half8, u32x4{h[0], h[1], h[2], h[3]});
+    lo = __builtin_bit_cast(half8, u32x4{l[0], l[1], l[2], l[3]});
+}
+__device__ __forceinline__ void split4(const float (&v)[4], half4& hi, half4& lo) {
+    uint32_t h[2], l[2];
+#pragma unroll
+    for (int j = 0; j < 2; ++j) split_pair(v[2 * j], v[2 * j + 1], h[j], l[j]);
+    typedef uint32_t u32x2 __attribute__((ext_vector_type(2)));
+    hi = __builtin_bit_cast(half4, u32x2{h[0], h[1]});
+    lo = __builtin_bit_cast(half4, u32x2{l[0], l[1]});
+}
+}
+
+namespace {
+struct X3Block {
+    static constexpr int C = 256, NW = 8, NE = 1, CK = 16 * NW * NE, NTHR = 64 * NW, NJ = C / 16 / NW;
+    static constexpr int XROW = C + 16;
+    static constexpr int TROW = CK + 16;
+    static constexpr size_t dws_bytes = size_t(NW) * NE * 1024;
+    static constexpr int T2BUF = NE == 1 ? 2 : 1;
+    static constexpr size_t lds_bytes = (size_t(2) * 64 * XROW + size_t(2) * T2BUF * 64 * TROW) * sizeof(half_t) + dws_bytes;
+};
+static_assert(X3Block::lds_bytes + 8192 <= 160 * 1024, "LDS budget (tower_p8_kernel<5> takes 8 KiB more for its records)");
+
+struct X3Tiles {
+    half_t *xh, *xl;
+    half_t *t2h, *t2l;
+    float* dws;
+};
+__device__ __forceinline__ X3Tiles x3_tiles(char* smem) {
+    X3Tiles t;
+    t.xh = reinterpret_cast<half_t*>(smem);
+    t.xl = t.xh + 64 * X3Block::XROW;
+    t.t2h = t.xl + 64 * X3Block::XROW;
+    t.t2l = t.t2h + X3Block::T2BUF * 64 * X3Block::TROW;
+    t.dws = reinterpret_cast<float*>(t.t2l + X3Block::T2BUF * 64 * X3Block::TROW);
+    return t;
+}
+
+__device__ __forceinline__ int x3_row(int sq) { return ((sq >> 3) & 3) * 16 + (sq >> 5) * 8 + (sq & 7); }
+__device__ __forceinline__ int x3_square(int row) { return ((row >> 4) + 4 * ((row >> 3) & 1)) * 8 + (row & 7); }
+
+typedef float f32x2 __attribute__((ext_vector_type(2)));
+template <int CTRL> __device__ __forceinline__ f32x2 dpp_mov2(f32x2 v) { return f32x2{dpp_mov<CTRL>(v.x), dpp_mov<CTRL>(v.y)}; }
+__device__ __forceinline__ f32x2 pair_of(const f32x4& v, int p) { return p == 0 ? f32x2{v[0], v[1]} : f32x2{v[2], v[3]}; }
+
+struct X3EdgeOffsets { int left, right; };
+__device__ __forceinline__ X3EdgeOffsets x3_edge_offsets(int l15) { return X3EdgeOffsets{(l15 & 7) == 0 ? 11 * 16 : 0, (l15 & 7) == 7 ? 5 * 16 : 0}; }
+struct X3Depthwise {
+    f32x2 w[11];
+    f32x2 S[6], L[6], R[6];
+    float outv[4][4];
+
+    template <int P> __device__ __forceinline__ void load(const float* rec, int lg, const X3EdgeOffsets& e) {
+#pragma unroll
+        for (int q = 0; q < 11; ++q) w[q] = *reinterpret_cast<const f32x2*>(rec + (q < 3 ? e.left : q >= 6 && q < 9 ? e.right : 0) + q * 16 + lg * 4 + 2 * P);
+    }
+    template <int P, bool SCALED = false> __device__ __forceinline__ void gather(const f32x4 (&acc)[4], bool upper, int c0 = 0, int c1 = 2, float acc_scale = 1.f) {
+        if constexpr (X3_ABL & 1) {
+#pragma unroll
+            for (int t = 0; t < 4; ++t) S[1 + t] = pair_of(acc[t], P) + w[0];
+            return;
+        }
+#pragma unroll
+        for (int c = 0; c < 2; ++c) {
+            if (c < c0 || c >= c1) continue;
+#pragma unroll
+            for (int t = 0; t < 4; ++t) S[1 + t][c] = SCALED ? fmaxf(fmaf(acc[t][2 * P + c], acc_scale, w[9][c]), 0.f) : fmaxf(acc[t][2 * P + c] + w[9][c], 0.f);
+            const float across_up = dpp_mov<DPP_ROW_ROR8>(S[4][c]), across_dn = dpp_mov<DPP_ROW_ROR8>(S[1][c]);
+            S[0][c] = upper ? across_up : 0.f;
+            S[5][c] = upper ? 0.f : across_dn;
+#pragma unroll
+            for (int j = 0; j < 6; ++j) {
+                L[j][c] = dpp_mov<DPP_ROW_SHR1>(S[j][c]);
+                R[j][c] = dpp_mov<DPP_ROW_SHL1>(S[j][c]);
+            }
+        }
+    }
+    template <int P> __device__ __forceinline__ void taps(int t0, int t1) {
+#pragma unroll
+        for (int t = 0; t < 4; ++t) {
+            if (t < t0 || t >= t1) continue;
+#pragma unroll
+            for (int c = 0; c < 2; ++c) {
+                if constexpr (X3_ABL & 1) {
+                    outv[t][2 * P + c] = S[1 + t][c];
+                    continue;
+                }
+                float a = w[10][c];
+#pragma unroll
+                for (int dy = 0; dy < 3; ++dy) {
+                    a = fmaf(w[dy][c], L[t + dy][c], a);
+                    a = fmaf(w[3 + dy][c], S[t + dy][c], a);
+                    a = fmaf(w[6 + dy][c], R[t + dy][c], a);
+                }
+                outv[t][2 * P + c] = fmaxf(a, 0.f);
+            }
+        }
+    }
+    __device__ __forceinline__ void pin_taps(int t0, int t1, int P) {
+#pragma unroll
+        for (int t = 0; t < 4; ++t)
+#pragma unroll
+            for (int c = 0; c < 2; ++c)
+                if (t >= t0 && t < t1) asm volatile("" : "+v"(outv[t][2 * P + c]));
+    }
+};
+__device__ __forceinline__ void x3_depthwise(const f32x4 (&acc)[4], const float* rec, int lg, bool upper, const X3EdgeOffsets& e, float (&outv)[4][4]) {
+    X3Depthwise dw;
+    dw.template load<0>(rec, lg, e);
+    dw.template gather<0>(acc, upper);
+    dw.template taps<0>(0, 4);
+    dw.template load<1>(rec, lg, e);
+    dw.template gather<1>(acc, upper);
+    dw.template taps<1>(0, 4);
+#pragma unroll
+    for (int t = 0; t < 4; ++t)
+#pragma unroll
+        for (int r = 0; r < 4; ++r) outv[t][r] = dw.outv[t][r];
+}
+struct X3EdgeOffsets5 { int o[5]; };
+__device__ __forceinline__ X3EdgeOffsets5 x3_edge_offsets5(int l15) {
+    const int f = l15 & 7;
+    X3EdgeOffsets5 e;
+    e.o[0] = f < 2 ? 27 * 16 : 0;
+    e.o[1] = f < 1 ? 22 * 16 : 0;
+    e.o[2] = 0;
+    e.o[3] = f > 6 ? 12 * 16 : 0;
+    e.o[4] = f > 5 ? 7 * 16 : 0;
+    return e;
+}
+struct X3Depthwise5 {
+    float w[27];
+    float S[8];
+    float outv[4][4];
+
+    template <int CH> __device__ __forceinline__ void load(const float* rec, int lg, const X3EdgeOffsets5& e) {
+#pragma unroll
+        for (int q = 0; q < 27; ++q) w[q] = rec[(q < 25 ? e.o[q / 5] : 0) + q * 16 + lg * 4 + CH];
+    }
+    template <int CH> __device__ __forceinline__ void gather(const f32x4 (&acc)[4], bool upper, float acc_scale) {
+#pragma unroll
+        for (int t = 0; t < 4; ++t) S[2 + t] = fmaxf(fmaf(acc[t][CH], acc_scale, w[25]), 0.f);
+        const float u3 = dpp_mov<DPP_ROW_ROR8>(S[5]), u2 = dpp_mov<DPP_ROW_ROR8>(S[4]);
+        const float d0 = dpp_mov<DPP_ROW_ROR8>(S[2]), d1 = dpp_mov<DPP_ROW_ROR8>(S[3]);
+        S[1] = upper ? u3 : 0.f;
+        S[0] = upper ? u2 : 0.f;
+        S[6] = upper ? 0.f : d0;
+        S[7] = upper ? 0.f : d1;
+    }
+    template <int CH> __device__ __forceinline__ void taps() {
+        float a[4];
+#pragma unroll
+        for (int t = 0; t < 4; ++t) a[t] = w[26];
+#pragma unroll
+        for (int j = 0; j < 8; ++j) {
+            const float v[5] = {dpp_mov<DPP_ROW_SHR2>(S[j]), dpp_mov<DPP_ROW_SHR1>(S[j]), S[j], dpp_mov<DPP_ROW_SHL1>(S[j]), dpp_mov<DPP_ROW_SHL2>(S[j])};
+#pragma unroll
+            for (int t = 0; t < 4; ++t) {
+                const int dy = j - t;
+                if (dy < 0 || dy > 4) continue;
+#pragma unroll
+                for (int g = 0; g < 5; ++g) a[t] = fmaf(w[g * 5 + dy], v[g], a[t]);
+            }
+        }
+#pragma unroll
+        for (int t = 0; t < 4; ++t) outv[t][CH] = fmaxf(a[t], 0.f);
+    }
+};
+__device__ __forceinline__ void x3_stage_tile(const X3Tiles& T, const float* xb, const float* g, int tid) {
+    constexpr int C = X3Block::C, XROW = X3Block::XROW;
+#pragma unroll 1
+    for (int i = tid; i < 64 * (C / 8); i += X3Block::NTHR) {
+        const int sq = i / (C / 8), v = i - sq * (C / 8), r = x3_row(sq);
+        float f[8];
+        load8<float>(xb + size_t(sq) * C + v * 8, f);
+        if (g) {
+            float gv[8];
+            load8<float>(g + v * 8, gv);
+#pragma unroll
+            for (int j = 0; j < 8; ++j) f[j] *= gv[j];
+        }
+        half8 h, l;
+        split8(f, h, l);
+        *reinterpret_cast<half8*>(T.xh + r * XROW + v * 8) = h;
+        *reinterpret_cast<half8*>(T.xl + r * XROW + v * 8) = l;
+    }
+}
+
+struct X3Weights {
+    __amdgpu_buffer_rsrc_t w1h, w1l, w3h, w3l;
+    __amdgpu_buffer_rsrc_t dw;
+    int cop_pad;
+};
+__device__ __forceinline__ __amdgpu_buffer_rsrc_t x3_rsrc(const void* p) {
+    const uint64_t v = reinterpret_cast<uint64_t>(p);
+    const uint64_t u = (uint64_t(uint32_t(__builtin_amdgcn_readfirstlane(int(uint32_t(v >> 32))))) << 32) |
+                       uint32_t(__builtin_amdgcn_readfirstlane(int(uint32_t(v))));
+    return __builtin_amdgcn_make_buffer_rsrc(reinterpret_cast<void*>(u), 0, 0x7fffffff, 0x00020000);
+}
+__device__ __forceinline__ X3Weights x3_weights(const void* w1h, const void* w1l, const void* w3h, const void* w3l, const float* dwpk, int cop_pad) {
+    X3Weights W;
+    W.w1h = x3_rsrc(w1h); W.w1l = x3_rsrc(w1l); W.w3h = x3_rsrc(w3h); W.w3l = x3_rsrc(w3l);
+    W.dw = x3_rsrc(dwpk);
+    W.cop_pad = __builtin_amdgcn_readfirstlane(cop_pad);
+    return W;
+}
+__device__ __forceinline__ half8 x3_frag(__amdgpu_buffer_rsrc_t r, uint32_t lane_off, uint32_t frag) {
+    typedef uint32_t u32x4 __attribute__((ext_vector_type(4)));
+    return __builtin_bit_cast(half8, __builtin_amdgcn_raw_buffer_load_b128(r, lane_off, frag * 1024u, 0));
+}
+}
+
+namespace {
+__device__ __forceinline__ void x3_se_fcs(const X3TowerBlock& d, const float* se_mean, float* se_h, float* se_gate, const f32x4 (&wa)[16], const f32x4 (&wb)[16], int tid) {
+    constexpr int GRP = 36;
+    auto dot32 = [](const f32x4 (&w)[16], const float* v, float& s0, float& s1) {
+#pragma unroll
+        for (int k4 = 0; k4 < 8; ++k4) {
+            const f32x4 m = *reinterpret_cast<const f32x4*>(v + 4 * k4);
+            s0 = fmaf(w[2 * k4][0], m[0], s0); s1 = fmaf(w[2 * k4][1], m[0], s1);
+            s0 = fmaf(w[2 * k4][2], m[1], s0); s1 = fmaf(w[2 * k4][3], m[1], s1);
+            s0 = fmaf(w[2 * k4 + 1][0], m[2], s0); s1 = fmaf(w[2 * k4 + 1][1], m[2], s1);
+            s0 = fmaf(w[2 * k4 + 1][2], m[3], s0); s1 = fmaf(w[2 * k4 + 1][3], m[3], s1);
+        }
+    };
+    if (d.se_kind == 1) {
+        {
+            const int j2 = tid >> 3, kq = tid & 7;
+            float s0 = 0.f, s1 = 0.f;
+            dot32(wa, se_mean + kq * GRP, s0, s1);
+            s0 += dpp_mov<0x111>(s0); s1 += dpp_mov<0x111>(s1);
+            s0 += dpp_mov<0x112>(s0); s1 += dpp_mov<0x112>(s1);
+            s0 += dpp_mov<0x114>(s0); s1 += dpp_mov<0x114>(s1);
+            if (kq == 7) {
+                float* h = se_h + (j2 >> 4) * GRP + 2 * (j2 & 15);
+                h[0] = fmaxf(s0, 0.f);
+                h[1] = fmaxf(s1, 0.f);
+            }
+        }
+        __syncthreads();
+        {
+            const int c2 = tid >> 2, kq = tid & 3;
+            float s0 = 0.f, s1 = 0.f;
+            dot32(wb, se_h + kq * GRP, s0, s1);
+            s0 += dpp_mov<0x111>(s0); s1 += dpp_mov<0x111>(s1);
+            s0 += dpp_mov<0x112>(s0); s1 += dpp_mov<0x112>(s1);
+            if (kq == 3) {
+                se_gate[2 * c2] = hard_sigmoid(s0);
+                se_gate[2 * c2 + 1] = hard_sigmoid(s1);
+            }
+        }
+    } else {
+        const int c2 = tid >> 2, kq = tid & 3;
+        float s0 = 0.f, s1 = 0.f;
+        dot32(wa, se_mean + (2 * kq) * GRP, s0, s1);
+        dot32(wb, se_mean + (2 * kq + 1) * GRP, s0, s1);
+        s0 += dpp_mov<0x111>(s0); s1 += dpp_mov<0x111>(s1);
+        s0 += dpp_mov<0x112>(s0); s1 += dpp_mov<0x112>(s1);
+        if (kq == 3) {
+            se_gate[2 * c2] = hard_sigmoid(d.se_b[2 * c2] + s0);
+            se_gate[2 * c2 + 1] = hard_sigmoid(d.se_b[2 * c2 + 1] + s1);
+        }
+    }
+    __syncthreads();
+}
+__device__ __forceinline__ void x3_se_gate_from_mean(const X3TowerBlock& d, float* scratch, int tid) {
+    constexpr int GRP = 36;
+    f32x4 wa[16], wb[16];
+    auto load_thread_weights = [&](const float* base, f32x4 (&dst)[16]) {
+        const f32x4* pk = reinterpret_cast<const f32x4*>(base) + tid;
+#pragma unroll
+        for (int i = 0; i < 16; ++i) dst[i] = pk[i * 512];
+    };
+    load_thread_weights(d.se_w1t, wa);
+    load_thread_weights(d.se_kind == 1 ? d.se_w2t : d.se_w1t + size_t(16) * 512 * 4, wb);
+    __syncthreads();
+    x3_se_fcs(d, scratch, scratch + 8 * GRP, scratch + 12 * GRP, wa, wb, tid);
+}
+
+template <int NJ>
+__device__ __forceinline__ void x3_stream_load(f32x4 (&x)[NJ][4], const float* xb, int tile0, int l15, int lg) {
+#pragma unroll
+    for (int j = 0; j < NJ; ++j)
+#pragma unroll
+        for (int t = 0; t < 4; ++t) x[j][t] = *reinterpret_cast<const f32x4*>(xb + size_t(x3_square(t * 16 + l15)) * X3Block::C + (tile0 + j) * 16 + lg * 4);
+}
+template <int NJ>
+__device__ __forceinline__ void x3_stream_store(const f32x4 (&x)[NJ][4], float* yb, int tile0, int l15, int lg) {
+#pragma unroll
+    for (int j = 0; j < NJ; ++j)
+#pragma unroll
+        for (int t = 0; t < 4; ++t) *reinterpret_cast<f32x4*>(yb + size_t(x3_square(t * 16 + l15)) * X3Block::C + (tile0 + j) * 16 + lg * 4) = x[j][t];
+}
+template <int NJ>
+__device__ __forceinline__ void x3_stream_add_bias(f32x4 (&x)[NJ][4], const float* b3, int tile0, int lg) {
+#pragma unroll
+    for (int j = 0; j < NJ; ++j) {
+        const f32x4 bs = *reinterpret_cast<const f32x4*>(b3 + (tile0 + j) * 16 + lg * 4);
+#pragma unroll
+        for (int t = 0; t < 4; ++t) x[j][t] += bs;
+    }
+}
+template <int NJ>
+__device__ __forceinline__ void x3_stream_write_tiles(const X3Tiles& T, const f32x4 (&x)[NJ][4], int tile0, int l15, int lg) {
+#pragma unroll
+    for (int j = 0; j < NJ; ++j) {
+        const int co0 = (tile0 + j) * 16 + lg * 4;
+#pragma unroll
+        for (int t = 0; t < 4; ++t) {
+            const int rr = t * 16 + l15;
+            const float v[4] = {x[j][t][0], x[j][t][1], x[j][t][2], x[j][t][3]};
+            half4 h, l;
+            split4(v, h, l);
+            *reinterpret_cast<half4*>(T.xh + rr * X3Block::XROW + co0) = h;
+            *reinterpret_cast<half4*>(T.xl + rr * X3Block::XROW + co0) = l;
+        }
+    }
+}
+template <int NJ>
+__device__ __forceinline__ void x3_stream_se(const X3Tiles& T, const X3TowerBlock& d, f32x4 (&x)[NJ][4], float* scratch, int tile0, int tid) {
+    constexpr int GRP = 36;
+    const int lane = tid & 63, l15 = lane & 15, lg = lane >> 4;
+#pragma unroll
+    for (int j = 0; j < NJ; ++j) {
+        float sum[4];
+#pragma unroll
+        for (int r = 0; r < 4; ++r) sum[r] = (x[j][0][r] + x[j][1][r]) + (x[j][2][r] + x[j][3][r]);
+#pragma unroll
+        for (int r = 0; r < 4; ++r) {
+            sum[r] += dpp_mov<0x111>(sum[r]);
+            sum[r] += dpp_mov<0x112>(sum[r]);
+            sum[r] += dpp_mov<0x114>(sum[r]);
+            sum[r] += dpp_mov<0x118>(sum[r]);
+        }
+        if (l15 == 15) {
+            const int c = (tile0 + j) * 16 + lg * 4;
+#pragma unroll
+            for (int r = 0; r < 4; ++r) scratch[((c + r) >> 5) * GRP + ((c + r) & 31)] = sum[r] * (1.f / 64.f);
+        }
+    }
+    x3_se_gate_from_mean(d, scratch, tid);
+    const float* se_gate = scratch + 12 * GRP;
+#pragma unroll
+    for (int j = 0; j < NJ; ++j) {
+        const f32x4 g = *reinterpret_cast<const f32x4*>(se_gate + (tile0 + j) * 16 + lg * 4);
+#pragma unroll
+        for (int t = 0; t < 4; ++t) x[j][t] *= g;
+    }
+    x3_stream_write_tiles<NJ>(T, x, tile0, l15, lg);
+    __syncthreads();
+}
+}
+
+}
diff --git a/crazyara_amd/csrc/nn/x3_tail.cpp b/crazyara_amd/csrc/nn/x3_tail.cpp
--- /dev/null
+++ b/crazyara_amd/csrc/nn/x3_tail.cpp
@@ -0,0 +1,335 @@
+#include "x3_device.h"
+
+#include <type_traits>
+
+namespace cra {
+
+template <int KS>
+__global__ __launch_bounds__(512) void tower_x3_tail_kernel(const X3TowerArgs a) {
+    static_assert(KS == 3 || KS == 5, "depthwise 3x3 or 5x5 (X3Depthwise / X3Depthwise5)");
+    constexpr int REC = KS == 3 ? 256 : 512;
+    using G = X3Block;
+    static_assert(G::NE == 1 && G::T2BUF == 2 && G::CK == 128, "the role kernel uses the NE = 1 tile geometry (two t2 buffers of 128 channels)");
+    constexpr int C = G::C, CK = G::CK, XROW = G::XROW, TROW = G::TROW;
+    extern __shared__ __attribute__((aligned(16))) char smem[];
+    const X3Tiles T = x3_tiles(smem);
+    const int b = blockIdx.x;
+    const int tid = threadIdx.x, lane = tid & 63, l15 = lane & 15, lg = lane >> 4;
+    const int wave = __builtin_amdgcn_readfirstlane(tid >> 6);
+    const bool expand_role = wave < 4;
+    const int w = wave & 3;
+    const uint32_t lane_off = uint32_t(lane) * 16u;
+    x3_stage_tile(T, a.x + size_t(b) * 64 * C, nullptr, tid);
+    __syncthreads();
+    constexpr int EW = 2;
+    half8 e_h[EW][2], e_l[EW][2];
+    bool first_chunk_requested = false;
+    if (expand_role) {
+    for (int blk = 0; blk < a.nblocks; ++blk) {
+        const X3TowerBlock& d = a.blocks[blk];
+        if (blk > 0 && d.se_kind != 0) {
+            x3_se_gate_from_mean(d, reinterpret_cast<float*>(T.t2h), tid);
+            __syncthreads();
+            first_chunk_requested = false;
+#pragma unroll
+            for (int ne = 0; ne < 2; ++ne) {
+#pragma unroll
+                for (int q = 0; q < EW; ++q) { asm volatile("" : "=v"(e_h[q][ne])); asm volatile("" : "=v"(e_l[q][ne])); }
+            }
+        }
+        const X3Weights W = x3_weights(d.w1pk, d.w1pk_lo, d.w3pk, d.w3pk_lo, d.dwpk, d.cop_pad);
+        const int n = W.cop_pad / CK;
+        const bool tail = __builtin_amdgcn_readfirstlane(d.tail) != 0;
+#ifdef CRA_X3_TRACE
+        const bool tracing = (b == 0 || b == 131) && blk == CRA_X3_TRACE;
+        int trace_n = 0;
+#endif
+        {
+            const bool hi = l15 >= 8;
+            const X3EdgeOffsets edge = x3_edge_offsets(l15);
+            auto e_tile = [&](int i, int ne) { return i * (CK / 16) + (tail && i == n - 1 ? w : w * 2 + ne); };
+            auto load_e = [&](auto one_c, int i, int s) {
+                if constexpr (X3_ABL & 16) return;
+#pragma unroll
+                for (int ne = 0; ne < (decltype(one_c)::value ? 1 : 2); ++ne) {
+                    const uint32_t f = uint32_t(e_tile(i, ne)) * (C / 32) + uint32_t(s);
+                    e_h[s % EW][ne] = x3_frag(W.w1h, lane_off, f);
+                    e_l[s % EW][ne] = x3_frag(W.w1l, lane_off, f);
+                }
+            };
+            auto load_first_chunk = [&](const X3Weights& Wx, bool one) {
+                if constexpr (X3_ABL & 16) return;
+#pragma unroll
+                for (int s = 0; s < EW; ++s)
+#pragma unroll
+                    for (int ne = 0; ne < 2; ++ne) {
+                        const uint32_t f = uint32_t(one ? w : w * 2 + ne) * (C / 32) + uint32_t(s);
+                        e_h[s][ne] = x3_frag(Wx.w1h, lane_off, f);
+                        e_l[s][ne] = x3_frag(Wx.w1l, lane_off, f);
+                    }
+            };
+            if constexpr (X3_ABL & 16) {
+#pragma unroll
+                for (int s = 0; s < EW; ++s)
+#pragma unroll
+                    for (int ne = 0; ne < 2; ++ne) e_h[s][ne] = e_l[s][ne] = *reinterpret_cast<const half8*>(T.xh + lane * 8);
+            }
+            if (!first_chunk_requested) load_first_chunk(W, tail && n == 1);
+            float* const my_dws = T.dws + (w * 2) * REC;
+            f32x4 accE[2][4], accD[2][4];
+            X3Depthwise dw;
+            X3Depthwise5 dw5;
+            const X3EdgeOffsets5 edge5 = x3_edge_offsets5(l15);
+            auto interval = [&](auto hase_c, auto hasd_c, auto onee_c, auto oned_c, int i) {
+                constexpr bool HASE = decltype(hase_c)::value, HASD = decltype(hasd_c)::value;
+                constexpr bool ONEE = decltype(onee_c)::value, ONED = decltype(oned_c)::value;
+                static_assert(!(ONEE && !HASE) && !(ONED && (HASE || !HASD)), "the tail chunk is expanded in interval n - 1 and runs the depthwise alone in interval n");
+                constexpr int NEE = ONEE ? 1 : 2;
+                half8 ring_h[4], ring_l[4];
+                auto read_step = [&](int st) {
+                    if constexpr (X3_ABL & 8) {
+                        ring_h[st % 4] = e_h[0][0];
+                        ring_l[st % 4] = e_l[0][0];
+                    } else {
+                        ring_h[st % 4] = *reinterpret_cast<const half8*>(T.xh + ((st & 3) * 16 + l15) * XROW + (st >> 2) * 32 + lg * 8);
+                        ring_l[st % 4] = *reinterpret_cast<const half8*>(T.xl + ((st & 3) * 16 + l15) * XROW + (st >> 2) * 32 + lg * 8);
+                    }
+                };
+                f32x4 dw_raw[NEE][REC / 256];
+                if constexpr (HASE) {
+#pragma unroll
+                    for (int ne = 0; ne < NEE; ++ne)
+#pragma unroll
+                        for (int h2 = 0; h2 < REC / 256; ++h2)
+                            dw_raw[ne][h2] = __builtin_bit_cast(f32x4, __builtin_amdgcn_raw_buffer_load_b128(W.dw, lane_off, uint32_t(e_tile(i, ne) * 16) * uint32_t(REC / 4) + uint32_t(h2) * 1024u, 0));
+#pragma unroll
+                    for (int ne = 0; ne < NEE; ++ne)
+#pragma unroll
+                        for (int t = 0; t < 4; ++t) accE[ne][t] = f32x4{0.f, 0.f, 0.f, 0.f};
+                    read_step(0); read_step(1); read_step(2);
+                }
+                if constexpr (HASD && KS == 3) dw.template load<0>(my_dws, lg, edge);
+                half_t* const t2h = T.t2h + ((i - 1) & 1) * 64 * TROW;
+                half_t* const t2l = T.t2l + ((i - 1) & 1) * 64 * TROW;
+#pragma unroll
+                for (int sl = 0; sl < (ONED ? C / 64 : C / 32); ++sl) {
+                    const int dt = sl / 4, ph = sl % 4;
+                    if constexpr (HASD) {
+                        if constexpr (KS == 3) {
+                            if (ph == 2) dw.template load<1>(my_dws + dt * 256, lg, edge);
+                            if (sl == 4) dw.template load<0>(my_dws + 256, lg, edge);
+                        } else {
+                            if (ph == 0) dw5.template load<0>(my_dws + dt * REC, lg, edge5);
+                            if (ph == 1) dw5.template load<1>(my_dws + dt * REC, lg, edge5);
+                            if (ph == 2) dw5.template load<2>(my_dws + dt * REC, lg, edge5);
+                            if (ph == 3) dw5.template load<3>(my_dws + dt * REC, lg, edge5);
+                        }
+                    }
+                    __builtin_amdgcn_sched_barrier(0);
+                    if constexpr (HASE) {
+#pragma unroll
+                        for (int t = 0; t < 4; ++t) {
+                            const int st = sl * 4 + t;
+                            if (st + 3 < 4 * (C / 32)) read_step(st + 3);
+#pragma unroll
+                            for (int ne = 0; ne < NEE; ++ne) {
+                                x3_mfma(e_l[sl % EW][ne], ring_h[st % 4], accE[ne][t], !(X3_ABL & 2));
+                                x3_mfma(e_h[sl % EW][ne], ring_l[st % 4], accE[ne][t], !(X3_ABL & 2));
+                                x3_mfma(e_h[sl % EW][ne], ring_h[st % 4], accE[ne][t], !(X3_ABL & 2));
+                            }
+                        }
+                        if (sl + EW < C / 32) load_e(onee_c, i, sl + EW);
+                        else if constexpr (ONEE) load_e(onee_c, i, sl + EW - C / 32);
+                        else load_e(onee_c, i + 1 < n ? i + 1 : i, sl + EW - C / 32);
+                    }
+                    if constexpr (HASD) {
+                        if constexpr (KS == 3) {
+                            if (ph == 0) dw.template gather<0>(accD[dt], hi);
+                            if (ph == 1) { dw.template taps<0>(0, 4); dw.pin_taps(0, 4, 0); }
+                            if (ph == 2) dw.template gather<1>(accD[dt], hi);
+                        } else {
+                            if (ph == 0) { dw5.template gather<0>(accD[dt], hi, 1.f); dw5.template taps<0>(); }
+                            if (ph == 1) { dw5.template gather<1>(accD[dt], hi, 1.f); dw5.template taps<1>(); }
+                            if (ph == 2) { dw5.template gather<2>(accD[dt], hi, 1.f); dw5.template taps<2>(); }
+                            if (ph == 3) { dw5.template gather<3>(accD[dt], hi, 1.f); dw5.template taps<3>(); }
+                        }
+                        if (ph == 3) {
+                            if constexpr (KS == 3) dw.template taps<1>(0, 4);
+                            const int cl = (ONED ? w : w * 2 + dt) * 16 + lg * 4;
+#pragma unroll
+                            for (int t = 0; t < 4; ++t) {
+                                half4 h, l;
+                                split4(KS == 3 ? dw.outv[t] : dw5.outv[t], h, l);
+                                if constexpr (X3_ABL & 64) {
+                                    asm volatile("" ::"v"(h), "v"(l));
+                                } else {
+                                    *reinterpret_cast<half4*>(t2h + (t * 16 + l15) * TROW + cl) = h;
+                                    *reinterpret_cast<half4*>(t2l + (t * 16 + l15) * TROW + cl) = l;
+                                }
+                            }
+                        }
+                    }
+                    if constexpr (HASE && HASD) {
+#pragma unroll
+                        for (int r = 0; r < 12 * NEE; ++r) {
+                            __builtin_amdgcn_sched_group_barrier(0x008, 1, 0);
+                            __builtin_amdgcn_sched_group_barrier(0x002, ONEE ? 8 : 4, 0);
+                        }
+                    }
+                    __builtin_amdgcn_sched_barrier(0);
+                }
+                if constexpr (HASE) {
+#pragma unroll
+                    for (int ne = 0; ne < NEE; ++ne)
+#pragma unroll
+                        for (int h2 = 0; h2 < REC / 256; ++h2) *reinterpret_cast<f32x4*>(my_dws + ne * REC + h2 * 256 + lane * 4) = dw_raw[ne][h2];
+#pragma unroll
+                    for (int ne = 0; ne < NEE; ++ne)
+#pragma unroll
+                        for (int t = 0; t < 4; ++t) accD[ne][t] = accE[ne][t];
+                }
+            };
+            constexpr std::true_type yes{};
+            constexpr std::false_type no{};
+            auto run = [&](auto hase_c, auto hasd_c, auto onee_c, auto oned_c, int i) {
+                const int kk = i - 1;
+                X3_STAMP(0);
+                interval(hase_c, hasd_c, onee_c, oned_c, i);
+                X3_STAMP(3);
+                if constexpr (!(X3_ABL & 32)) __syncthreads();
+                X3_STAMP(4);
+            };
+            const int nfull = tail ? n - 1 : n;
+            if (nfull == 0) run(yes, no, yes, no, 0);
+            else run(yes, no, no, no, 0);
+            for (int i = 1; i < nfull; ++i) run(yes, yes, no, no, i);
+            if (tail) {
+                if (nfull > 0) run(yes, yes, yes, no, n - 1);
+                run(no, yes, no, yes, n);
+            } else run(no, yes, no, no, n);
+            first_chunk_requested = false;
+            if (blk + 1 < a.nblocks && a.blocks[blk + 1].se_kind == 0) {
+                const X3TowerBlock& dn = a.blocks[blk + 1];
+                load_first_chunk(x3_weights(dn.w1pk, dn.w1pk_lo, dn.w3pk, dn.w3pk_lo, dn.dwpk, dn.cop_pad), dn.tail != 0 && dn.cop_pad == CK);
+                first_chunk_requested = true;
+            }
+            __syncthreads();
+            { const int kk = n; X3_STAMP(5); }
+        }
+    }
+    } else {
+    constexpr int NJ = 4;
+    f32x4 accX[NJ][4];
+    x3_stream_load<NJ>(accX, a.x + size_t(b) * 64 * C, w * NJ, l15, lg);
+    for (int blk = 0; blk < a.nblocks; ++blk) {
+        const X3TowerBlock& d = a.blocks[blk];
+        if (blk > 0 && d.se_kind != 0) x3_stream_se<NJ>(T, d, accX, reinterpret_cast<float*>(T.t2h), w * NJ, tid);
+        const X3Weights W = x3_weights(d.w1pk, d.w1pk_lo, d.w3pk, d.w3pk_lo, d.dwpk, d.cop_pad);
+        const int n = W.cop_pad / CK;
+        const int nslab3 = W.cop_pad >> 5;
+        const bool tail = __builtin_amdgcn_readfirstlane(d.tail) != 0;
+#ifdef CRA_X3_TRACE
+        const bool tracing = (b == 0 || b == 131) && blk == CRA_X3_TRACE;
+        int trace_n = 0;
+#endif
+        {
+            constexpr int PW = 2;
+            half8 p_h[PW][NJ], p_l[PW][NJ];
+            auto load_p = [&](int k, int s2) {
+                if constexpr (X3_ABL & 16) return;
+#pragma unroll
+                for (int j = 0; j < NJ; ++j) {
+                    const uint32_t f = uint32_t(w * NJ + j) * uint32_t(nslab3) + uint32_t(k * (CK / 32) + s2);
+                    p_h[s2 % PW][j] = x3_frag(W.w3h, lane_off, f);
+                    p_l[s2 % PW][j] = x3_frag(W.w3l, lane_off, f);
+                }
+            };
+            if constexpr (X3_ABL & 16) {
+#pragma unroll
+                for (int s2 = 0; s2 < PW; ++s2)
+#pragma unroll
+                    for (int j = 0; j < NJ; ++j) p_h[s2][j] = p_l[s2][j] = *reinterpret_cast<const half8*>(T.xl + lane * 8);
+            }
+            x3_stream_add_bias<NJ>(accX, d.b3, w * NJ, lg);
+#pragma unroll
+            for (int s2 = 0; s2 < PW; ++s2) load_p(0, s2);
+            if constexpr (!(X3_ABL & 32)) {
+                __syncthreads();
+                __syncthreads();
+            }
+            auto project = [&](auto one_c, int kk) {
+                constexpr int NS2 = decltype(one_c)::value ? CK / 64 : CK / 32;
+                const half_t* const t2h = T.t2h + (kk & 1) * 64 * TROW;
+                const half_t* const t2l = T.t2l + (kk & 1) * 64 * TROW;
+                X3_STAMP(8);
+                half8 bh[2][4], bl[2][4];
+                auto read_t2 = [&](int s2, half8 (&h)[4], half8 (&l)[4]) {
+#pragma unroll
+                    for (int t = 0; t < 4; ++t) {
+                        if constexpr (X3_ABL & 8) {
+                            h[t] = p_h[s2 % PW][0];
+                            l[t] = p_l[s2 % PW][0];
+                        } else {
+                            h[t] = *reinterpret_cast<const half8*>(t2h + (t * 16 + l15) * TROW + s2 * 32 + lg * 8);
+                            l[t] = *reinterpret_cast<const half8*>(t2l + (t * 16 + l15) * TROW + s2 * 32 + lg * 8);
+                        }
+                    }
+                };
+                read_t2(0, bh[0], bl[0]);
+#pragma unroll
+                for (int s2 = 0; s2 < NS2; ++s2) {
+                    if (s2 + 1 < NS2) read_t2(s2 + 1, bh[(s2 + 1) & 1], bl[(s2 + 1) & 1]);
+                    __builtin_amdgcn_sched_barrier(0);
+#pragma unroll
+                    for (int j = 0; j < NJ; ++j)
+#pragma unroll
+                        for (int t = 0; t < 4; ++t) x3_mfma(p_l[s2 % PW][j], bh[s2 & 1][t], accX[j][t], !(X3_ABL & 4));
+#pragma unroll
+                    for (int j = 0; j < NJ; ++j)
+#pragma unroll
+                        for (int t = 0; t < 4; ++t) x3_mfma(p_h[s2 % PW][j], bl[s2 & 1][t], accX[j][t], !(X3_ABL & 4));
+#pragma unroll
+                    for (int j = 0; j < NJ; ++j)
+#pragma unroll
+                        for (int t = 0; t < 4; ++t) x3_mfma(p_h[s2 % PW][j], bh[s2 & 1][t], accX[j][t], !(X3_ABL & 4));
+                    if (s2 + PW < NS2) load_p(kk, s2 + PW);
+                    else if constexpr (decltype(one_c)::value) load_p(kk, s2 + PW - NS2);
+                    else load_p(kk + 1 < n ? kk + 1 : kk, s2 + PW - NS2);
+                    if (s2 == 1) X3_STAMP(9);
+                    __builtin_amdgcn_sched_barrier(0);
+                }
+                X3_STAMP(10);
+            };
+            const int nfull = tail ? n - 1 : n;
+            for (int kk = 0; kk < nfull; ++kk) {
+                project(std::false_type{}, kk);
+                if (kk + 1 < n) {
+                    if constexpr (!(X3_ABL & 32)) __syncthreads();
+                }
+                X3_STAMP(11);
+            }
+            if (tail) {
+                const int kk = n - 1;
+                project(std::true_type{}, kk);
+                X3_STAMP(11);
+            }
+            if (blk + 1 < a.nblocks && a.blocks[blk + 1].se_kind == 0) x3_stream_write_tiles<NJ>(T, accX, w * NJ, l15, lg);
+            { const int kk = n; X3_STAMP(12); }
+            __syncthreads();
+            { const int kk = n; X3_STAMP(13); }
+        }
+    }
+    x3_stream_store<NJ>(accX, a.y + size_t(b) * 64 * C, w * NJ, l15, lg);
+    }
+}
+
+void init_x3_tail_kernel_attributes() {
+    (void)hipFuncSetAttribute(reinterpret_cast<const void*>(&tower_x3_tail_kernel<3>), hipFuncAttributeMaxDynamicSharedMemorySize, int(X3Block::lds_bytes));
+    (void)hipFuncSetAttribute(reinterpret_cast<const void*>(&tower_x3_tail_kernel<5>), hipFuncAttributeMaxDynamicSharedMemorySize, int(X3Block::lds_bytes + 8192));
+}
+void launch_tower_x3_tail(const X3TowerArgs& a, hipStream_t s) {
+    if (a.ks == 5) hipLaunchKernelGGL(tower_x3_tail_kernel<5>, dim3(a.batch), dim3(X3Block::NTHR), X3Block::lds_bytes + 8192, s, a);
+    else hipLaunchKernelGGL(tower_x3_tail_kernel<3>, dim3(a.batch), dim3(X3Block::NTHR), X3Block::lds_bytes, s, a);
+}
+
+}
```

Measured after the change: 347,800 evals/s (median of 6 runs). 1.02x the previous value.
